# Hawkeye-FineGrained/Hawkeye

Hardware: AMD Instinct MI355X
Metric: images/sec (train fwd+bwd) BCNN VGG-16 448^2 bs64 (higher is better)
Workload: dtype f32; 1 GPU; BCNN_S2: VGG-16 448x448, per-GPU batch 64, 200 classes, SGD momentum 0.9, CE label_smoothing 0.1, full train step; global_batch=64, parallelism=dp1, memory_format=channels_last

## Files before the change

hawkeye_amd/_lib.py:

```python
import ctypes
import os

import torch

_HERE = os.path.dirname(os.path.abspath(__file__))
LIB_PATH = os.path.join(_HERE, 'csrc', 'libhawkeye_hip.so')

c_f = ctypes.c_void_p
c_i = ctypes.c_int
c_sz = ctypes.c_size_t
c_ll = ctypes.c_longlong
c_fl = ctypes.c_float

SIGNATURES = {
    'hk_version': (ctypes.c_char_p, []),
    'hk_tuning_set': (c_i, [ctypes.c_char_p, c_i]),
    'hk_tuning_get': (c_i, [ctypes.c_char_p, ctypes.POINTER(ctypes.c_int)]),
    'hk_bcnn_pool_ws_bytes': (c_sz, [c_i, c_i, c_i]),
    'hk_bcnn_pool_fwd': (c_i, [c_f, c_f, c_f, c_f, c_i, c_i, c_i, c_f, c_sz, c_f]),
    'hk_bcnn_pool_bwd': (c_i, [c_f, c_f, c_f, c_f, c_f, c_f, c_i, c_i, c_i, c_f, c_sz, c_f]),
    'hk_bcnn_pool_bwd_tdot': (c_i, [c_f, c_f, c_f, c_f, c_f, c_f, c_f, c_f, c_i, c_f, c_i, c_i, c_i, c_f, c_sz, c_f]),
    'hk_bcnn_ssqrt_ws_bytes': (c_sz, [c_i, c_i, c_i]),
    'hk_bcnn_ssqrt_pool_fwd': (c_i, [c_f, c_f, c_f, c_i, c_i, c_i, c_f, c_sz, c_f]),
    'hk_bcnn_ssqrt_pool_bwd': (c_i, [c_f, c_f, c_f, c_f, c_f, c_i, c_i, c_i, c_f, c_sz, c_f]),
    'hk_bcnn_ssqrt_pool_fwd_parts': (c_i, [c_f, c_f, c_f, ctypes.c_void_p, c_i, c_i, c_i, c_f]),
    'hk_linear_fwd_ssq': (c_i, [c_f, c_f, c_f, c_f, c_i, c_f, c_f, c_i, c_i, c_i, c_f, c_sz, c_f]),
    'hk_bcnn_ssqrt_pool_bwd_tdot': (c_i, [c_f, c_f, c_f, c_f, c_f, c_f, c_f, c_i, c_i, c_f, c_i, c_i, c_i, c_f, c_sz, c_f]),
    'hk_bcnn_ssqrt_pool_fwd_unscaled': (c_i, [c_f, c_f, c_f, c_i, c_i, c_i, c_f, c_sz, c_f]),
    'hk_bcnn_ssqrt_pool_bwd_unscaled': (c_i, [c_f, c_f, c_f, c_f, c_f, c_i, c_i, c_i, c_f, c_sz, c_f]),
    'hk_bcnn_colsum_norm': (c_i, [c_f, c_f, c_f, c_i, c_i, c_i, c_f, c_sz, c_f]),
    'hk_bcnn_gram_norm': (c_i, [c_f, c_f, c_f, c_i, c_i, c_i, c_f]),
    'hk_bcnn_bwd_gemm': (c_i, [c_f, c_f, c_f, c_f, c_f, c_f, c_i, c_i, c_i, c_f]),
    'hk_bcnn_bwd_rank1': (c_i, [c_f, c_f, c_f, c_f, c_i, c_i, c_i, c_f]),
    'hk_cov_pool_fwd': (c_i, [c_f, c_f, c_f, c_i, c_i, c_i, c_f]),
    'hk_cov_pool_bwd': (c_i, [c_f, c_f, c_f, c_f, c_i, c_i, c_i, c_f]),
    'hk_ns_sqrtm_ws_bytes': (c_sz, [c_i, c_i, c_i, c_i]),
    'hk_ns_sqrtm_fwd': (c_i, [c_f, c_f, c_f, c_f, c_f, c_i, c_i, c_i, c_f, c_sz, c_f]),
    'hk_ns_sqrtm_fwd_sym': (c_i, [c_f, c_f, c_f, c_f, c_f, c_i, c_i, c_i, c_f, c_sz, c_f]),
    'hk_ns_sqrtm_triu_fwd': (c_i, [c_f, c_f, c_f, c_f, c_f, c_f, c_i, c_i, c_i, c_i, c_f, c_sz, c_f]),
    'hk_ns_sqrtm_bwd': (c_i, [c_f, c_f, c_f, c_f, c_f, c_f, c_f, c_i, c_i, c_i, c_f, c_sz, c_f]),
    'hk_ns_sqrtm_bwd_general': (c_i, [c_f, c_f, c_f, c_f, c_f, c_f, c_f, c_i, c_i, c_i, c_f, c_sz, c_f]),
    'hk_triu_vec_fwd': (c_i, [c_f, c_f, c_i, c_i, c_f]),
    'hk_triu_vec_bwd': (c_i, [c_f, c_f, c_i, c_i, c_f]),
    'hk_cbp_plan_bytes': (c_sz, [c_i, c_i]),
    'hk_cbp_plan_build': (c_i, [c_f, c_f, c_f, c_f, c_i, c_i, c_f, c_f]),
    'hk_cbp_plan_destroy': (c_i, [c_f]),
    'hk_cbp_ws_bytes': (c_sz, [c_i, c_i, c_i, c_i]),
    'hk_cbp_fwd': (c_i, [c_f, c_f, c_f, c_f, c_f, c_i, c_i, c_i, c_i, c_f, c_sz, c_f]),
    'hk_cbp_bwd': (c_i, [c_f, c_f, c_f, c_f, c_f, c_f, c_f, c_i, c_i, c_i, c_i, c_f, c_sz, c_f]),
    'hk_trunk_ws_bytes': (c_sz, [c_i]),
    'hk_bias_relu_fwd': (c_i, [c_f, c_f, c_f, c_ll, c_i, c_f]),
    'hk_bias_relu_bwd': (c_i, [c_f, c_f, c_f, c_f, c_f, c_ll, c_i, c_f, c_sz, c_f]),
    'hk_bias_relu_pool_fwd': (c_i, [c_f, c_f, c_f, c_f, c_i, c_i, c_i, c_i, c_f]),
    'hk_bias_relu_pool_bwd': (c_i, [c_f, c_f, c_f, c_f, c_f, c_i, c_i, c_i, c_i, c_f, c_sz, c_f]),
    'hk_conv1_ws_bytes': (c_sz, [c_i]),
    'hk_conv1_bias_relu_fwd': (c_i, [c_f, c_f, c_f, c_f, c_f, c_i, c_i, c_i, c_i, c_i, c_f]),
    'hk_conv1_bias_relu_bwd': (c_i, [c_f, c_f, c_f, c_f, c_f, c_i, c_i, c_i, c_i, c_i, c_f, c_sz, c_f]),
    'hk_conv3x3_wrw_ws_bytes': (c_sz, [c_i, c_i]),
    'hk_conv3x3_wrw': (c_i, [c_f, c_f, c_f, c_i, c_i, c_i, c_i, c_i, c_f, c_sz, c_f]),
    'hk_add_relu_fwd': (c_i, [c_f, c_f, c_ll, c_f]),
    'hk_relu_mask_bwd': (c_i, [c_f, c_f, c_f, c_ll, c_f]),
    'hk_cbp_rect_plan_bytes': (c_sz, [c_i, c_i, c_i]),
    'hk_cbp_rect_plan_build': (c_i, [c_f, c_f, c_i, c_f, c_f, c_i, c_i, c_f, c_f]),
    'hk_cbp_rect_bin_matrix': (c_i, [c_f, c_f, c_f, c_i, c_i, c_i, c_i, c_f]),
    'hk_cbp_rect_unbin_matrix': (c_i, [c_f, c_f, c_f, c_i, c_i, c_i, c_i, c_f]),
    'hk_cbp_rect_loc_fwd': (c_i, [c_f, c_f, c_f, c_f, c_i, c_i, c_i, c_i, c_i, c_f]),
    'hk_cbp_rect_loc_bwd': (c_i, [c_f, c_f, c_f, c_f, c_f, c_f, c_i, c_i, c_i, c_i, c_i, c_f]),
    'hk_att_pool_fwd': (c_i, [c_f, c_f, c_f, c_f, c_i, c_i, c_i, c_f]),
    'hk_att_pool_bwd': (c_i, [c_f, c_f, c_f, c_f, c_f, c_f, c_i, c_i, c_i, c_f]),
    'hk_att_pool3_fwd': (c_i, [c_f] * 8 + [c_i] * 5 + [c_f]),
    'hk_att_pool3_bwd': (c_i, [c_f] * 14 + [c_i] * 5 + [c_f]),
    'hk_att_roi_select3': (c_i, [c_f, c_f, c_f, c_i, c_f, c_f, c_f, c_f, c_i, c_i, c_f, c_fl, c_f, c_f]),
    'hk_att_roi_select': (c_i, [c_f, c_f, c_f, c_i, c_i, c_i, c_i, c_fl, c_i, c_i, c_i, c_i, c_i, c_i, c_fl, c_i, c_f]),
    'hk_roi_crop_resize_fwd': (c_i, [c_f, c_f, c_f, c_f, c_i, c_i, c_i, c_i, c_i, c_f]),
    'hk_roi_crop_resize_bwd': (c_i, [c_f, c_f, c_f, c_f, c_i, c_i, c_i, c_i, c_i, c_f]),
    'hk_roi_boxes': (c_i, [c_f, c_f, c_i, c_f, c_f, c_i, c_f, c_f, c_i, c_f, c_fl, c_f, c_f, c_i, c_f]),
    'hk_osme_gap': (c_i, [c_f, c_f, c_i, c_i, c_i, c_f]),
    'hk_osme_scale_fwd': (c_i, [c_f, c_f, c_f, c_i, c_i, c_i, c_i, c_f]),
    'hk_osme_scale_bwd': (c_i, [c_f, c_f, c_f, c_f, c_f, c_f, c_i, c_i, c_i, c_i, c_f]),
    'hk_linear_ws_bytes': (c_sz, [c_i, c_i, c_i]),
    'hk_linear_fwd': (c_i, [c_f, c_f, c_f, c_f, c_i, c_i, c_i, c_f, c_sz, c_f]),
    'hk_linear_bwd': (c_i, [c_f, c_f, c_f, c_f, c_f, c_f, c_i, c_i, c_i, c_f]),
    'hk_linear_fwd_scaled': (c_i, [c_f, c_f, c_f, c_f, c_f, c_i, c_i, c_i, c_f, c_sz, c_f]),
    'hk_linear_bwd_scaled': (c_i, [c_f, c_f, c_f, c_f, c_f, c_f, c_f, c_i, c_i, c_i, c_f]),
    'hk_npairs_ws_bytes': (c_sz, [c_i, c_i]),
    'hk_npairs_loss': (c_i, [c_f, c_f, c_f, c_f, c_i, c_i, c_i, c_f, c_sz, c_f]),
    'hk_peer_loss_ws_bytes': (c_sz, [c_i, c_i]),
    'hk_peer_loss': (c_i, [c_f, c_f, c_f, ctypes.c_double, c_f, c_f, c_f, c_f, c_i, c_i, c_f, c_sz, c_f]),
    'hk_api_pairs': (c_i, [c_f, c_f, c_f, c_i, c_i, c_f]),
    'hk_api_gather_fwd': (c_i, [c_f, c_f, c_f, c_i, c_i, c_f]),
    'hk_api_gather_bwd': (c_i, [c_f, c_f, c_f, c_i, c_i, c_f]),
    'hk_api_interact_fwd': (c_i, [c_f, c_f, c_f, c_f, c_fl, c_f, c_i, c_i, c_f]),
    'hk_api_interact_bwd': (c_i, [c_f, c_f, c_f, c_f, c_fl, c_f, c_f, c_f, c_i, c_i, c_f]),
    'hk_apinet_loss_ws_bytes': (c_sz, [c_i, c_i]),
    'hk_apinet_loss': (c_i, [c_f, c_f, c_f, c_fl, c_fl, c_f, c_f, c_f, c_i, c_i, c_f, c_sz, c_f]),
    'hk_nts_nms': (c_i, [c_f, c_f, c_f, c_f, c_i, c_i, c_i, ctypes.c_double, c_f]),
    'hk_nts_crop_resize': (c_i, [c_f, c_f, c_f] + [c_i] * 8 + [c_f]),
    'hk_nts_loss_ws_bytes': (c_sz, [c_i, c_i, c_i]),
    'hk_nts_loss': (c_i, [c_f] * 5 + [c_fl] + [c_f] * 5 + [c_i, c_i, c_i, c_f, c_sz, c_f]),
    'hk_crossx_me_fwd': (c_i, [c_f] * 7 + [c_i] * 5 + [c_f]),
    'hk_crossx_me_bwd': (c_i, [c_f] * 12 + [c_i] * 5 + [c_f]),
    'hk_crossx_up_add_fwd': (c_i, [c_f] * 3 + [c_i] * 6 + [c_f]),
    'hk_crossx_up_add_bwd': (c_i, [c_f] * 2 + [c_i] * 6 + [c_f]),
    'hk_crossx_loss_ws_bytes': (c_sz, [c_i] * 6),
    'hk_crossx_loss': (c_i, [c_f] * 7 + [c_fl] * 4 + [c_f] * 7 + [c_i] * 6 + [c_f, c_sz, c_f]),
    'hk_cin_sci_fwd': (c_i, [c_f, c_f, c_f, c_i, c_i, c_i, c_f]),
    'hk_cin_sci_bwd': (c_i, [c_f, c_f, c_f, c_f, c_i, c_f, c_i, c_i, c_i, c_f]),
    'hk_cin_cci_fwd': (c_i, [c_f, c_f, c_f, c_f, c_i, c_i, c_i, c_f]),
    'hk_cin_cci_ws_bytes': (c_sz, [c_i, c_i]),
    'hk_cin_cci_bwd': (c_i, [c_f, c_f, c_f, c_f, c_f, c_f, c_f, c_i, c_i, c_i, c_f, c_sz, c_f]),
    'hk_image_finalize': (c_i, [c_f, c_f, c_f, c_f, c_f, c_i, c_i, c_i, c_i, c_f]),
    'hk_bgemm_f32': (c_i, [c_f, c_i, c_ll, c_i, c_f, c_i, c_ll, c_i, c_f, c_i, c_ll, c_i, c_i, c_i, c_i,
                           c_fl, c_fl, c_fl, c_f]),
    'hk_dcl_head_fwd_ws_bytes': (c_sz, [c_i] * 4),
    'hk_dcl_head_fwd': (c_i, [c_f] * 5 + [c_i] * 4 + [c_f, c_sz, c_f]),
    'hk_dcl_head_bwd_ws_bytes': (c_sz, [c_i] * 4),
    'hk_dcl_head_bwd': (c_i, [c_f] * 8 + [c_i] * 4 + [c_f, c_sz, c_f]),
    'hk_dcl_loss': (c_i, [c_f] * 6 + [c_fl] * 5 + [c_f] * 4 + [c_i] * 4 + [c_f]),
    'hk_dcl_swap_law': (c_i, [c_f] * 6 + [c_i] * 5 + [c_f]),
}

TRUNK_SIGNATURES = {
    'hk_conv3x3_ws_bytes': (c_sz, [c_i, c_i]),
    'hk_conv3x3_fwd': (c_i, [c_f, c_f, c_f, c_i, c_i, c_i, c_i, c_i, c_f, c_sz, c_f]),
    'hk_conv3x3_bwd_data': (c_i, [c_f, c_f, c_f, c_i, c_i, c_i, c_i, c_i, c_f, c_sz, c_f]),
}

TRUNK_EPI_SIGNATURES = {
    'hk_conv3x3_bias_relu_fwd': (c_i, [c_f, c_f, c_f, c_f, c_f, c_i, c_i, c_i, c_i, c_i, c_f, c_sz, c_f]),
    'hk_conv3x3_bias_relu_pool_fwd': (c_i, [c_f, c_f, c_f, c_f, c_f, c_i, c_i, c_i, c_i, c_i, c_f, c_sz, c_f]),
    'hk_conv3x3_masked_ws_bytes': (c_sz, [c_i, c_i, c_i, c_i, c_i]),
    'hk_conv3x3_masked_bwd_data': (c_i, [c_f, c_f, c_f, c_f, c_f, c_i, c_i, c_i, c_i, c_i, c_f, c_sz, c_f]),
}

TRUNK_TILE_SIGNATURES = {
    'hk_conv3x3_tile_plan': (c_i, [c_i, c_i, c_i, c_i, c_f]),
}

TRUNK_POOL_SIGNATURES = {
    'hk_conv3x3_wrw_pooled': (c_i, [c_f, c_f, c_f, c_f, c_f, c_i, c_i, c_i, c_i, c_i, c_f, c_sz, c_f]),
    'hk_conv3x3_wrw_pooled_served': (c_i, [c_i] * 5),
    'hk_conv3x3_wrw_pooled_plan': (c_i, [c_i] * 5 + [c_f]),
}

INTERP_SIGNATURES = {
    'hk_ip_group_fwd_ws_bytes': (c_sz, [c_i] * 5),
    'hk_ip_group_fwd': (c_i, [c_f] * 7 + [c_i] * 5 + [c_f, c_sz, c_f]),
    'hk_ip_group_bwd_ws_bytes': (c_sz, [c_i] * 5),
    'hk_ip_group_bwd': (c_i, [c_f] * 11 + [c_i] * 5 + [c_f, c_sz, c_f]),
    'hk_ip_loss_ws_bytes': (c_sz, [c_i, c_i]),
    'hk_ip_loss': (c_i, [c_f] * 5 + [c_fl] + [c_f] * 3 + [c_i] * 6 + [c_f, c_sz, c_f]),
}

MGE_SIGNATURES = {
    'hk_mge_partpool_fwd_ws_bytes': (c_sz, [c_i] * 5),
    'hk_mge_partpool_fwd': (c_i, [c_f] * 5 + [c_i] * 5 + [c_f, c_sz, c_f]),
    'hk_mge_partpool_bwd': (c_i, [c_f] * 6 + [c_i] * 5 + [c_f]),
    'hk_mge_cam_bbox': (c_i, [c_f] * 4 + [c_i] * 5 + [c_fl, c_i, c_f]),
    'hk_mge_loss_ws_bytes': (c_sz, [c_i, c_i]),
    'hk_mge_loss': (c_i, [c_f, c_f, c_fl, c_f, c_f, c_i, c_i, c_i, c_f, c_sz, c_f]),
}


def attach(lib):
    for name, (res, args) in list(SIGNATURES.items()) + list(TRUNK_SIGNATURES.items()) + list(TRUNK_EPI_SIGNATURES.items()) + \
            list(TRUNK_TILE_SIGNATURES.items()) + list(TRUNK_POOL_SIGNATURES.items()) + list(INTERP_SIGNATURES.items()) + list(MGE_SIGNATURES.items()):
        fn = getattr(lib, name)
        fn.restype = res
        fn.argtypes = args
    return lib


_lib = None


HK_OK, HK_ERR_BAD_ARG, HK_ERR_WORKSPACE, HK_ERR_UNSUPPORTED = 0, -1, -2, -3


class HawkeyeHipError(RuntimeError):
    pass


def load():
    global _lib
    if _lib is not None:
        return _lib
    if not os.path.exists(LIB_PATH):
        raise HawkeyeHipError(
            f'{LIB_PATH} not found: build it with `python -c "import __graft_entry__ as g; g.build()"` '
            f'or `make -C hawkeye_amd/csrc` (there is no CPU fallback for the HIP ops)')
    _lib = attach(ctypes.CDLL(LIB_PATH, mode=ctypes.RTLD_GLOBAL))
    return _lib


def check(rc, what):
    if rc != 0:
        raise HawkeyeHipError(f'{what} failed with code {rc} '
                              f'({"HK_ERR" if rc < 0 else "hipError_t"})')


def ptr(t):
    if t is None:
        return None
    if not t.is_cuda:
        raise HawkeyeHipError('hawkeye_amd ops run on MI355X only: got a CPU tensor (no CPU fallback; '
                              'the CPU reference lives in oracle/ and is test infrastructure)')
    if not (t.is_contiguous() or (t.dim() == 4 and t.is_contiguous(memory_format=torch.channels_last))):
        raise HawkeyeHipError('internal error: non-contiguous tensor handed to the C ABI')
    if t.device.index != torch.cuda.current_device():
        raise HawkeyeHipError(f'tensor lives on {t.device} but the current HIP device is cuda:{torch.cuda.current_device()}: '
                              f'call torch.cuda.set_device({t.device.index}) (one process per GPU) or wrap the call in '
                              f'`with torch.cuda.device(...)`')
    return ctypes.c_void_p(t.data_ptr())


class tuning:

    def __init__(self, **knobs):
        self.knobs = knobs
        self.saved = {}

    def __enter__(self):
        lib = load()
        for name, value in self.knobs.items():
            old = ctypes.c_int(0)
            check(lib.hk_tuning_get(name.encode(), ctypes.byref(old)), f'hk_tuning_get({name})')
            self.saved[name] = old.value
            check(lib.hk_tuning_set(name.encode(), int(value)), f'hk_tuning_set({name})')
        return self

    def __exit__(self, *exc):
        lib = load()
        for name, value in self.saved.items():
            lib.hk_tuning_set(name.encode(), value)
        return False


def stream():
    return ctypes.c_void_p(torch.cuda.current_stream().cuda_stream)
```

hawkeye_amd/csrc/api.hip:

```cpp
#include <cstdlib>
#include <cstring>

#include "hk_bgemm.h"
#include "../../include/hawkeye_hip.h"

namespace hk {

namespace {
struct Knob {
    const char* name;
    const char* env;
    int Tuning::*field;
};
const Knob kKnobs[] = {
    {"bcnn_generic", "HK_BCNN_GENERIC", &Tuning::bcnn_generic}, {"cbp_bin", "HK_CBP_BIN", &Tuning::cbp_bin},
    {"roi_bwd", "HK_ROI_BWD", &Tuning::roi_bwd},                {"linear_slabs", "HK_LINEAR_SLABS", &Tuning::linear_slabs},
    {"ns_tn", "HK_NS_TN", &Tuning::ns_tn},                      {"bwd_v", "HK_BWD_V", &Tuning::bwd_v},
    {"ns_streams", "HK_NS_STREAMS", &Tuning::ns_streams},        {"sched_b", "HK_SCHED_B", &Tuning::sched_b},
    {"ns_sym", "HK_NS_SYM", &Tuning::ns_sym},
    {"lin_walk", "HK_LIN_WALK", &Tuning::lin_walk},           {"bwd_fold", "HK_BWD_FOLD", &Tuning::bwd_fold},
    {"fwd_fold", "HK_FWD_FOLD", &Tuning::fwd_fold},             {"conv_wrw", "HK_CONV_WRW", &Tuning::conv_wrw},
    {"wrw_wgs", "HK_WRW_WGS", &Tuning::wrw_wgs},                {"peer_form", "HK_PEER_FORM", &Tuning::peer_form},
    {"wrw_split", "HK_WRW_SPLIT", &Tuning::wrw_split},          {"wrw_wide", "HK_WRW_WIDE", &Tuning::wrw_wide},
    {"conv_fwd", "HK_CONV_FWD", &Tuning::conv_fwd},             {"conv_bwd_data", "HK_CONV_BWD_DATA", &Tuning::conv_bwd_data},
    {"conv_epi", "HK_CONV_EPI", &Tuning::conv_epi},             {"conv_mfma", "HK_CONV_MFMA", &Tuning::conv_mfma},
    {"wrw_mfma", "HK_WRW_MFMA", &Tuning::wrw_mfma},             {"conv_tile", "HK_CONV_TILE", &Tuning::conv_tile},
    {"wrw_pool", "HK_WRW_POOL", &Tuning::wrw_pool},
};
Tuning from_env() {
    Tuning t;
    for (const Knob& k : kKnobs)
        if (const char* e = getenv(k.env)) t.*(k.field) = atoi(e);
    return t;
}
}

Tuning& tuning() {
    static Tuning t = from_env();
    return t;
}

}

using namespace hk;

extern "C" int hk_tuning_set(const char* name, int value) {
    if (!name) return HK_ERR_BAD_ARG;
    for (const Knob& k : kKnobs)
        if (!strcmp(name, k.name)) {
            tuning().*(k.field) = value;
            return HK_OK;
        }
    return HK_ERR_BAD_ARG;
}

extern "C" int hk_tuning_get(const char* name, int* value) {
    if (!name || !value) return HK_ERR_BAD_ARG;
    for (const Knob& k : kKnobs)
        if (!strcmp(name, k.name)) {
            *value = tuning().*(k.field);
            return HK_OK;
        }
    return HK_ERR_BAD_ARG;
}

extern "C" const char* hk_version(void) { return "hawkeye_hip 0.1 gfx950"; }

extern "C" int hk_bgemm_f32(const float* a, int lda, long long stride_a, int trans_a, const float* b, int ldb,
                            long long stride_b, int trans_b, float* c, int ldc, long long stride_c, int M, int N,
                            int K, int batch, float alpha, float beta, float diag, hk_stream_t stream) {
    if (!a || !b || !c) return HK_ERR_BAD_ARG;
    hipStream_t st = (hipStream_t)stream;
    const LdPlain la = trans_a ? make_plain(a, stride_a, lda, K, M) : make_plain(a, stride_a, lda, M, K);
    const LdPlain lb = trans_b ? make_plain(b, stride_b, ldb, N, K) : make_plain(b, stride_b, ldb, K, N);
    const EpAffine ep = make_affine(c, stride_c, ldc, alpha, nullptr, beta, diag);
    if (!trans_a && !trans_b) return bgemm_launch<true, false>(la, lb, ep, M, N, K, batch, st);
    if (!trans_a && trans_b) return bgemm_launch<true, true>(la, lb, ep, M, N, K, batch, st);
    if (trans_a && !trans_b) return bgemm_launch<false, false>(la, lb, ep, M, N, K, batch, st);
    return bgemm_launch<false, true>(la, lb, ep, M, N, K, batch, st);
}
```

hawkeye_amd/csrc/conv_fwd.hip:

```cpp
#include "hk_common.h"
#include "hk_split_bf16.h"
#include <hk_mfma_bf16.h>
#include "../../include/hawkeye_hip.h"

namespace hk {

constexpr int CF_CO = 64;
constexpr int CF_R = 4;
constexpr int CF_SW = 32;
constexpr int CF_CK = 32;
constexpr int CF_PIX = 80;
constexpr int CF_HW = CF_SW + 2;
constexpr int CF_HPIX = (CF_R + 2) * CF_HW;
constexpr int CF_XPLANE = CF_HPIX * CF_PIX;
constexpr int CF_WPLANE = CF_CO * CF_PIX;
constexpr int CF_WTAP = 3 * CF_WPLANE;
constexpr int CF_LDS = 3 * CF_XPLANE + 2 * CF_WTAP;
constexpr int CF_XF4 = CF_HPIX * (CF_CK / 4);
constexpr int CF_XU = (CF_XF4 + 255) / 256;
constexpr int CF_FLUSH = 3;

constexpr int CF_MF_32 = 0, CF_MF_16 = 1;
constexpr int CF16_PIX = 64;
constexpr int CF16_XPLANE = CF_HPIX * CF16_PIX;
constexpr int CF16_WPLANE = CF_CO * CF16_PIX;
constexpr int CF16_WTAP = 3 * CF16_WPLANE;
constexpr int CF16_LDS = 3 * CF16_XPLANE + 2 * CF16_WTAP;

constexpr int CF_G_4x32 = 0, CF_G_8x16 = 1, CF_G_16x8 = 2;
template <int G>
struct CfGeo {
    static constexpr int TH = G == CF_G_4x32 ? 4 : (G == CF_G_8x16 ? 8 : 16), TW = 128 / TH;
    static constexpr int HR = TH + 2, HC = TW + 2;
    static constexpr int HP = G == CF_G_16x8 ? 16 : HC;
    static constexpr int LPIX = HR * HP;
    static constexpr int XF4 = HR * HC * (CF_CK / 4);
    static constexpr int XU = (XF4 + 255) / 256;
    static constexpr int PBD = G == CF_G_4x32 ? 16 : (G == CF_G_8x16 ? HP : 2 * HP);
    __host__ __device__ static constexpr int trow(bool m32, int wave, int pb, int l) {
        return G == CF_G_4x32 ? wave : (G == CF_G_8x16 ? 2 * wave + (m32 ? l >> 4 : pb) : 4 * wave + 2 * pb + (l >> 3));
    }
    __host__ __device__ static constexpr int tcol(bool m32, int pb, int l) {
        return G == CF_G_4x32 ? (m32 ? l : 16 * pb + l) : (G == CF_G_8x16 ? (m32 ? (l < 16 ? l : (l - 2) & 15) : l) : l & 7);
    }
};
static_assert(CfGeo<CF_G_4x32>::LPIX == CF_HPIX && CfGeo<CF_G_4x32>::XU == CF_XU && CfGeo<CF_G_4x32>::HP == CF_HW, "4 x 32 is the tile above");
constexpr int CF_PLAN_4x32 = 0, CF_PLAN_8x16 = 1, CF_PLAN_MIXED = 2;
template <int MF, int G>
constexpr int cf_xplane() { return CfGeo<G>::LPIX * (MF == CF_MF_32 ? CF_PIX : CF16_PIX); }
template <int MF, int PLAN>
constexpr int cf_lds() {
    return 3 * cf_xplane<MF, PLAN == CF_PLAN_MIXED ? CF_G_16x8 : PLAN>() + 2 * (MF == CF_MF_32 ? CF_WTAP : CF16_WTAP);
}
static_assert(cf_lds<CF_MF_32, CF_PLAN_4x32>() == CF_LDS && cf_lds<CF_MF_16, CF_PLAN_4x32>() == CF16_LDS, "4 x 32 keeps its LDS");
static_assert(cf_lds<CF_MF_32, CF_PLAN_8x16>() <= CF_LDS && cf_lds<CF_MF_16, CF_PLAN_MIXED>() == 79872 && 2 * 79872 <= 160 * 1024,
              "two workgroups per CU with every plan");
#define CF_TAP_BARRIER(n)                                                                                      \
    do {                                                                                                       \
        asm volatile("" ::: "memory");                                         \
        __builtin_amdgcn_s_waitcnt(HK_VMCNT_IMM(n) & ~(15 << 8));                                              \
        __builtin_amdgcn_s_barrier();                                                                          \
        asm volatile("" ::: "memory");                                                                         \
    } while (0)
__host__ __device__ constexpr int cf16_off(int row, int kg) { return row * CF16_PIX + ((kg ^ ((row >> 1) & 2)) << 4); }
constexpr int CF_B128_GROUPS[4][16] = {{0, 1, 2, 3, 12, 13, 14, 15, 20, 21, 22, 23, 24, 25, 26, 27},
                                       {4, 5, 6, 7, 8, 9, 10, 11, 16, 17, 18, 19, 28, 29, 30, 31},
                                       {32, 33, 34, 35, 44, 45, 46, 47, 52, 53, 54, 55, 56, 57, 58, 59},
                                       {36, 37, 38, 39, 40, 41, 42, 43, 48, 49, 50, 51, 60, 61, 62, 63}};
template <int G>
constexpr bool cf16_group_conflict_free(int g) {
    constexpr int LAST = CfGeo<G>::trow(false, 0, 0, 15) * CfGeo<G>::HP + CfGeo<G>::tcol(false, 0, 15);
    for (int base = 0; base + LAST < CfGeo<G>::LPIX; ++base) {
        unsigned seen = 0;
        for (int i = 0; i < 16; ++i) {
            const int lane = CF_B128_GROUPS[g][i], l = lane & 15;
            const int pix = base + CfGeo<G>::trow(false, 0, 0, l) * CfGeo<G>::HP + CfGeo<G>::tcol(false, 0, l);
            const int slot = (cf16_off(pix, lane >> 4) >> 4) & 15;
            if ((seen >> slot) & 1u) return false;
            seen |= 1u << slot;
        }
    }
    return true;
}
template <int G>
constexpr bool cf16_conflict_free() {
    return cf16_group_conflict_free<G>(0) && cf16_group_conflict_free<G>(1) && cf16_group_conflict_free<G>(2) && cf16_group_conflict_free<G>(3);
}
static_assert(cf16_conflict_free<CF_G_4x32>() && cf16_conflict_free<CF_G_8x16>() && cf16_conflict_free<CF_G_16x8>(),
              "every ds_read_b128 lane group of a CF_MF_16 fragment reads 16 different slots, in every geometry at its pitch");
template <int G>
constexpr bool cf32_conflict_free() {
    for (int g = 0; g < 4; ++g)
        for (int base = 0; base + CfGeo<G>::HP + 16 < CfGeo<G>::LPIX; ++base) {
            unsigned seen = 0;
            for (int i = 0; i < 16; ++i) {
                const int lane = CF_B128_GROUPS[g][i], l = lane & 31;
                const int pix = base + CfGeo<G>::trow(true, 0, 0, l) * CfGeo<G>::HP + CfGeo<G>::tcol(true, 0, l);
                const int slot = ((pix * CF_PIX + (lane >> 5) * 16) >> 4) & 15;
                if ((seen >> slot) & 1u) return false;
                seen |= 1u << slot;
            }
        }
    return true;
}
static_assert(cf32_conflict_free<CF_G_4x32>() && cf32_conflict_free<CF_G_8x16>(), "the CF_MF_32 pixel fragment, both geometries");
static_assert(cf16_off(16, 1) == cf16_off(0, 1) + 16 * CF16_PIX && cf16_off(35, 2) == cf16_off(3, 2) + 32 * CF16_PIX,
              "rows 16 and 32 further on are a constant offset away");
static_assert(CF16_WTAP <= CF_WTAP && CF16_WTAP == 3 * 256 * 16, "the workspace holds either image; a weight tile is three loads a thread");

template <int MF>
__global__ __launch_bounds__(256) void conv3x3_wsplit_kernel(const float* __restrict__ w, char* __restrict__ ws, int M, int K,
                                                             int transposed, long long total) {
    const long long i = (long long)blockIdx.x * 256 + threadIdx.x;
    if (i >= total) return;
    const int nchunk = K / CF_CK;
    constexpr int NQ = MF == CF_MF_32 ? 10 : 8;
    const int q = (int)(i % NQ);
    long long r = i / NQ;
    const int co = (int)(r % CF_CO);
    r /= CF_CO;
    const int tap = (int)(r % 9);
    const int chunk = (int)((r / 9) % nchunk), cot = (int)((r / 9) / nchunk);
    const long long m = (long long)cot * CF_CO + co, k0 = (long long)chunk * CF_CK + 4 * q;
    f32x4 v = {0.f, 0.f, 0.f, 0.f};
    if (q < 8) {
        if (!transposed) {
            v = *reinterpret_cast<const f32x4*>(w + (m * 9 + tap) * K + k0);
        } else {
#pragma unroll
            for (int e = 0; e < 4; ++e) v[e] = w[((k0 + e) * 9 + (8 - tap)) * M + m];
        }
    }
    bf16x4 p[3];
    wrs_split(v, p);
    if (MF == CF_MF_32) {
        char* d = ws + (size_t)r * CF_WTAP + co * CF_PIX + q * 8;
#pragma unroll
        for (int s = 0; s < 3; ++s) *reinterpret_cast<bf16x4*>(d + s * CF_WPLANE) = p[s];
    } else {
        char* d = ws + (size_t)r * CF16_WTAP + cf16_off(co, q >> 1) + (q & 1) * 8;
#pragma unroll
        for (int s = 0; s < 3; ++s) *reinterpret_cast<bf16x4*>(d + s * CF16_WPLANE) = p[s];
    }
}

__device__ __forceinline__ bf16x8 cf_frag(const char* p) {
#if defined(__HIP_DEVICE_COMPILE__)
    return *(const __attribute__((address_space(3))) bf16x8*)p;
#else
    bf16x8 f;
    __builtin_memcpy(&f, p, 16);
    return f;
#endif
}

constexpr int CF_EPI_NONE = 0, CF_EPI_RELU = 1, CF_EPI_POOL = 2, CF_EPI_MASK = 3;
constexpr int CF_PARK = CF_CO + 4;
constexpr int CF_DB_RPG = 128;
static_assert(CF_R * CF_SW * CF_PARK * 4 <= CF_LDS, "the parked tile fits the LDS of the main loop");

__device__ __forceinline__ f32x4 cf_relu4(f32x4 v) {
    f32x4 r;
#pragma unroll
    for (int t = 0; t < 4; ++t) r[t] = v[t] < 0.f ? 0.f : v[t];
    return r;
}
__device__ __forceinline__ unsigned cf_sign4(f32x4 r) {
    return (!(r[0] <= 0.f) ? 1u : 0u) | (!(r[1] <= 0.f) ? 2u : 0u) | (!(r[2] <= 0.f) ? 4u : 0u) | (!(r[3] <= 0.f) ? 8u : 0u);
}

template <int EPI, int G>
__device__ __forceinline__ void cf16_epilogue(const f32x4 (&acc4)[4][2], const f32x4 (&sum4)[4][2], float* ldsf, float* __restrict__ y, int H,
                                              int W, int Cout, long long n, int r0, int c0, int cot, int tile, int wave, int tid, int l15,
                                              int kg, const float* __restrict__ bias, uint8_t* __restrict__ mk,
                                              double* __restrict__ part) {
    typedef CfGeo<G> GE;
    const int c4 = Cout / 4;
    bool live[2];
    long long pix[2];
    f32x4 v[4][2];
#pragma unroll
    for (int pb = 0; pb < 2; ++pb) {
        const int row = r0 + GE::trow(false, wave, pb, l15), col = c0 + GE::tcol(false, pb, l15);
        live[pb] = row < H && col < W;
        pix[pb] = (n * H + row) * W + col;
#pragma unroll
        for (int cb = 0; cb < 4; ++cb) v[cb][pb] = sum4[cb][pb] + acc4[cb][pb];
    }
    if (EPI == CF_EPI_RELU || EPI == CF_EPI_POOL) {
        const f32x4* b4 = reinterpret_cast<const f32x4*>(bias + cot * CF_CO + 4 * kg);
#pragma unroll
        for (int cb = 0; cb < 4; ++cb) {
            const f32x4 b = b4[4 * cb];
#pragma unroll
            for (int pb = 0; pb < 2; ++pb) v[cb][pb] = cf_relu4(v[cb][pb] + b);
        }
    }
    if (EPI == CF_EPI_MASK) {
        typedef unsigned u32x4 __attribute__((ext_vector_type(4)));
#pragma unroll
        for (int pb = 0; pb < 2; ++pb) {
            u32x4 mb = {0u, 0u, 0u, 0u};
            if (live[pb]) mb = *reinterpret_cast<const u32x4*>(mk + pix[pb] * c4 + cot * (CF_CO / 4));
#pragma unroll
            for (int cb = 0; cb < 4; ++cb) {
                const unsigned bits = mb[cb] >> (8 * kg);
#pragma unroll
                for (int e = 0; e < 4; ++e) v[cb][pb][e] = ((bits >> e) & 1u) != 0u ? v[cb][pb][e] : 0.f;
            }
        }
    }
    if (EPI != CF_EPI_POOL) {
#pragma unroll
        for (int pb = 0; pb < 2; ++pb)
            if (live[pb]) {
                float* yp = y + pix[pb] * Cout + cot * CF_CO + 4 * kg;
#pragma unroll
                for (int cb = 0; cb < 4; ++cb) *reinterpret_cast<f32x4*>(yp + 16 * cb) = v[cb][pb];
            }
    }
    if (EPI == CF_EPI_RELU) {
        if (mk) {
#pragma unroll
            for (int pb = 0; pb < 2; ++pb) {
                unsigned own = 0;
#pragma unroll
                for (int cb = 0; cb < 4; ++cb) own |= cf_sign4(v[cb][pb]) << (8 * cb);
                unsigned m4 = 0;
#pragma unroll
                for (int j = 0; j < 4; ++j) m4 |= ((__shfl(own, l15 + 16 * j) >> (8 * kg)) & 0xffu) << (8 * j);
                if (live[pb]) *reinterpret_cast<unsigned*>(mk + pix[pb] * c4 + cot * (CF_CO / 4) + 4 * kg) = m4;
            }
        }
    }
    if (EPI == CF_EPI_POOL) {
        float* park = ldsf;
#pragma unroll
        for (int pb = 0; pb < 2; ++pb) {
            float* mine = park + (GE::trow(false, wave, pb, l15) * GE::TW + GE::tcol(false, pb, l15)) * CF_PARK + 4 * kg;
#pragma unroll
            for (int cb = 0; cb < 4; ++cb) *reinterpret_cast<f32x4*>(mine + 16 * cb) = v[cb][pb];
        }
    }
    if (EPI == CF_EPI_MASK) {
        double s[16];
#pragma unroll
        for (int cb = 0; cb < 4; ++cb)
#pragma unroll
            for (int e = 0; e < 4; ++e) s[4 * cb + e] = (double)v[cb][0][e] + (double)v[cb][1][e];
#pragma unroll
        for (int d = 8; d >= 1; d >>= 1) {
            const bool up = (l15 & d) != 0;
#pragma unroll
            for (int i = 0; i < d; ++i) {
                const double send = up ? s[i] : s[i + d], keep = up ? s[i + d] : s[i];
                s[i] = keep + __shfl_xor(send, d);
            }
        }
        double* red = reinterpret_cast<double*>(ldsf);
        red[wave * CF_CO + 16 * (l15 >> 2) + 4 * kg + (l15 & 3)] = s[0];
        __syncthreads();
        if (tid < CF_CO)
            part[(long long)tile * Cout + cot * CF_CO + tid] = ((red[tid] + red[CF_CO + tid]) + red[2 * CF_CO + tid]) + red[3 * CF_CO + tid];
    }
}

template <int EPI, int MF, int G>
__device__ __forceinline__ void conv3x3_split_tile(float* ldsf, const float* __restrict__ x, const char* __restrict__ ws, float* __restrict__ y,
                                                   int H, int W, int Cin, int Cout, long long n, int r0, int c0, int tile, int cot,
                                                   const float* __restrict__ bias, uint8_t* __restrict__ mk, double* __restrict__ part) {
    typedef CfGeo<G> GE;
    constexpr bool M32 = MF == CF_MF_32;
    static_assert(!(M32 && G == CF_G_16x8), "16 x 8 is a geometry of CF_MF_16 only");
    constexpr int XPLANE = cf_xplane<MF, G>(), WTAP = M32 ? CF_WTAP : CF16_WTAP;
    constexpr int XU = GE::XU, XF4 = GE::XF4, HC = GE::HC, HP = GE::HP;
    char* xs = reinterpret_cast<char*>(ldsf);
    char* wb = xs + 3 * XPLANE;
    const int tid = threadIdx.x, lane = tid & 63, l31 = lane & 31, hf = lane >> 5;
    const int l15 = lane & 15, kg = lane >> 4;
    const int wave = __builtin_amdgcn_readfirstlane(tid >> 6);
    const int nchunk = Cin / CF_CK, total = nchunk * 9;
    const float* xi = x + n * H * W * Cin;
    const char* wt = ws + (size_t)cot * total * WTAP + tid * 16;

    long long xoff[XU];
    unsigned xok = 0;
#pragma unroll
    for (int u = 0; u < XU; ++u) {
        const int idx = tid + 256 * u;
        const bool in = idx < XF4;
        const int p = in ? idx >> 3 : 0, hr = p / HC, hc = p - hr * HC;
        const int row = r0 - 1 + hr, col = c0 - 1 + hc;
        if (in && row >= 0 && row < H && col >= 0 && col < W) xok |= 1u << u;
        const int rc = row < 0 ? 0 : (row < H ? row : H - 1), cc = col < 0 ? 0 : (col < W ? col : W - 1);
        xoff[u] = ((long long)rc * W + cc) * Cin + 4 * (idx & 7);
    }
    const int xdst = M32 ? (tid >> 3) * CF_PIX + (tid & 7) * 8 : cf16_off(tid >> 3, (tid & 7) >> 1) + (tid & 1) * 8;
    auto xdst_of = [&](int u) {
        if constexpr (HP == HC) {
            return xdst + u * 32 * (M32 ? CF_PIX : CF16_PIX);
        } else {
            const int p = (tid >> 3) + 32 * u, hr = p / HC;
            return cf16_off(hr * HP + (p - hr * HC), (tid & 7) >> 1) + (tid & 1) * 8;
        }
    };

    f32x4 vx[XU];
    auto load_x = [&](int chunk) {
        const float* b = xi + chunk * CF_CK;
#pragma unroll
        for (int u = 0; u < XU; ++u) HK_LOAD16_ASYNC(vx[u], b + xoff[u]);
    };
    auto load_w = [&](int it, int buf) {
        const char* b = wt + (size_t)it * WTAP;
        char* d = wb + buf * WTAP + wave * 1024;
#pragma unroll
        for (int u = 0; u < 3; ++u) glds16(reinterpret_cast<const float*>(b + 4096 * u), reinterpret_cast<float*>(d + 4096 * u));
        if constexpr (M32) {
            if (wave < 3) glds16(reinterpret_cast<const float*>(b + 3 * 4096), reinterpret_cast<float*>(d + 3 * 4096));
        }
    };
    auto store_x = [&]() {
        const f32x4 zero = {0.f, 0.f, 0.f, 0.f};
#pragma unroll
        for (int u = 0; u < XU; ++u) {
            if (tid + 256 * u < XF4) {
                bf16x4 p[3];
                wrs_split(((xok >> u) & 1) ? vx[u] : zero, p);
                const int d = xdst_of(u);
#pragma unroll
                for (int s = 0; s < 3; ++s) *reinterpret_cast<bf16x4*>(xs + s * XPLANE + d) = p[s];
            }
        }
    };

    f32x16 acc[2], sum[2];
    f32x4 acc4[4][2], sum4[4][2];
    if constexpr (M32) {
#pragma unroll
        for (int cb = 0; cb < 2; ++cb)
#pragma unroll
            for (int i = 0; i < 16; ++i) acc[cb][i] = sum[cb][i] = 0.f;
    } else {
#pragma unroll
        for (int cb = 0; cb < 4; ++cb)
#pragma unroll
            for (int pb = 0; pb < 2; ++pb)
#pragma unroll
                for (int e = 0; e < 4; ++e) acc4[cb][pb][e] = sum4[cb][pb][e] = 0.f;
    }

    load_w(0, 0);
    load_x(0);
    __builtin_amdgcn_s_waitcnt(HK_VMCNT_IMM(0));
#pragma unroll
    for (int u = 0; u < XU; ++u) HK_PIN_LOADED(vx[u]);
    store_x();
    HK_LDS_BARRIER();

    const int aoff = l31 * CF_PIX + hf * 16;
    const int boff = (GE::trow(true, wave, 0, l31) * HP + GE::tcol(true, 0, l31)) * CF_PIX + hf * 16;
    const int bpix = GE::trow(false, wave, 0, l15) * HP + GE::tcol(false, 0, l15);
    int since = 0;
    for (int chunk = 0; chunk < nchunk; ++chunk) {
        const bool more = chunk + 1 < nchunk;
#pragma unroll
        for (int tap = 0; tap < 9; ++tap) {
            const int it = chunk * 9 + tap;
            load_w(it + 1 < total ? it + 1 : it, (it + 1) & 1);
            if (tap == 5) load_x(more ? chunk + 1 : chunk);
            if constexpr (M32) {
            const char* A = wb + (it & 1) * CF_WTAP + aoff;
            const char* B = xs + boff + ((tap / 3) * HP + tap % 3) * CF_PIX;
            bf16x8 a[2][2][3], b[2][3];
#pragma unroll
            for (int ks = 0; ks < 2; ++ks)
#pragma unroll
                for (int s = 0; s < 3; ++s) {
                    b[ks][s] = cf_frag(B + s * XPLANE + ks * 32);
                    a[ks][0][s] = cf_frag(A + s * CF_WPLANE + ks * 32);
                    a[ks][1][s] = cf_frag(A + s * CF_WPLANE + 32 * CF_PIX + ks * 32);
                }
            __builtin_amdgcn_sched_barrier(0);
#pragma unroll
            for (int ks = 0; ks < 2; ++ks)
#pragma unroll
                for (int cb = 0; cb < 2; ++cb) {
                    acc[cb] = __builtin_amdgcn_mfma_f32_32x32x16_bf16(a[ks][cb][1], b[ks][1], acc[cb], 0, 0, 0);
                    acc[cb] = __builtin_amdgcn_mfma_f32_32x32x16_bf16(a[ks][cb][0], b[ks][2], acc[cb], 0, 0, 0);
                    acc[cb] = __builtin_amdgcn_mfma_f32_32x32x16_bf16(a[ks][cb][2], b[ks][0], acc[cb], 0, 0, 0);
                    acc[cb] = __builtin_amdgcn_mfma_f32_32x32x16_bf16(a[ks][cb][0], b[ks][1], acc[cb], 0, 0, 0);
                    acc[cb] = __builtin_amdgcn_mfma_f32_32x32x16_bf16(a[ks][cb][1], b[ks][0], acc[cb], 0, 0, 0);
                    acc[cb] = __builtin_amdgcn_mfma_f32_32x32x16_bf16(a[ks][cb][0], b[ks][0], acc[cb], 0, 0, 0);
                }
            } else {
                const char* A = wb + (it & 1) * CF16_WTAP + cf16_off(l15, kg);
                const int bp = bpix + (tap / 3) * HP + tap % 3;
                const char* Bp[2];
                Bp[0] = xs + cf16_off(bp, kg);
                Bp[1] = GE::PBD % 16 == 0 ? Bp[0] + GE::PBD * CF16_PIX : xs + cf16_off(bp + GE::PBD, kg);
                bf16x8 a[4][3], b[2][3];
#pragma unroll
                for (int s = 0; s < 3; ++s) {
#pragma unroll
                    for (int pb = 0; pb < 2; ++pb) b[pb][s] = cf_frag(Bp[pb] + s * XPLANE);
#pragma unroll
                    for (int cb = 0; cb < 4; ++cb) a[cb][s] = cf_frag(A + s * CF16_WPLANE + cb * 16 * CF16_PIX);
                }
                __builtin_amdgcn_sched_barrier(0);
                constexpr int PA[6] = {1, 0, 2, 0, 1, 0}, PB[6] = {1, 2, 0, 1, 0, 0};
#pragma unroll
                for (int pr = 0; pr < 6; ++pr)
#pragma unroll
                    for (int cb = 0; cb < 4; ++cb)
#pragma unroll
                        for (int pb = 0; pb < 2; ++pb) acc4[cb][pb] = mfma_f32_16x16x32_bf16(a[cb][PA[pr]], b[pb][PB[pr]], acc4[cb][pb]);
            }
            if (tap == 5) CF_TAP_BARRIER(XU);
            else CF_TAP_BARRIER(0);
            if (tap == 6) {
#pragma unroll
                for (int u = 0; u < XU; ++u) HK_PIN_LOADED(vx[u]);
            }
            if (tap == 8 && more) {
                store_x();
                HK_LDS_BARRIER();
            }
        }
        if (++since == CF_FLUSH) {
            if constexpr (M32) {
#pragma unroll
                for (int cb = 0; cb < 2; ++cb) {
                    sum[cb] += acc[cb];
#pragma unroll
                    for (int i = 0; i < 16; ++i) acc[cb][i] = 0.f;
                }
            } else {
#pragma unroll
                for (int cb = 0; cb < 4; ++cb)
#pragma unroll
                    for (int pb = 0; pb < 2; ++pb) {
                        sum4[cb][pb] += acc4[cb][pb];
#pragma unroll
                        for (int e = 0; e < 4; ++e) acc4[cb][pb][e] = 0.f;
                    }
            }
            since = 0;
        }
    }
    if constexpr (!M32) {
        cf16_epilogue<EPI, G>(acc4, sum4, ldsf, y, H, W, Cout, n, r0, c0, cot, tile, wave, tid, l15, kg, bias, mk, part);
        if (EPI != CF_EPI_POOL) return;
    }
    const int trow = GE::trow(true, wave, 0, l31), tcol = GE::tcol(true, 0, l31);
    const int row = r0 + trow, col = c0 + tcol;
    if (EPI == CF_EPI_NONE) {
        if (row < H && col < W) {
            float* yp = y + ((n * H + row) * W + col) * Cout + cot * CF_CO + 4 * hf;
#pragma unroll
            for (int cb = 0; cb < 2; ++cb)
#pragma unroll
                for (int j = 0; j < 4; ++j) {
                    f32x4 v;
#pragma unroll
                    for (int e = 0; e < 4; ++e) v[e] = sum[cb][4 * j + e] + acc[cb][4 * j + e];
                    *reinterpret_cast<f32x4*>(yp + cb * 32 + 8 * j) = v;
                }
        }
        return;
    }
    const bool live = row < H && col < W;
    const long long pix = (n * H + row) * W + col;
    const int c4 = Cout / 4;
    f32x4 v[2][4];
    if constexpr (M32) {
#pragma unroll
    for (int cb = 0; cb < 2; ++cb)
#pragma unroll
        for (int j = 0; j < 4; ++j)
#pragma unroll
            for (int e = 0; e < 4; ++e) v[cb][j][e] = sum[cb][4 * j + e] + acc[cb][4 * j + e];
    }
    if (M32 && (EPI == CF_EPI_RELU || EPI == CF_EPI_POOL)) {
        const f32x4* b4 = reinterpret_cast<const f32x4*>(bias + cot * CF_CO + 4 * hf);
#pragma unroll
        for (int cb = 0; cb < 2; ++cb)
#pragma unroll
            for (int j = 0; j < 4; ++j) v[cb][j] = cf_relu4(v[cb][j] + b4[8 * cb + 2 * j]);
    }
    if (EPI == CF_EPI_RELU) {
        if (live) {
            float* yp = y + pix * Cout + cot * CF_CO + 4 * hf;
#pragma unroll
            for (int cb = 0; cb < 2; ++cb)
#pragma unroll
                for (int j = 0; j < 4; ++j) *reinterpret_cast<f32x4*>(yp + cb * 32 + 8 * j) = v[cb][j];
        }
        if (mk) {
            unsigned own[2];
#pragma unroll
            for (int cb = 0; cb < 2; ++cb) {
                own[cb] = 0;
#pragma unroll
                for (int j = 0; j < 4; ++j) own[cb] |= cf_sign4(v[cb][j]) << (8 * j);
            }
            const unsigned theirs0 = __shfl_xor(own[0], 32), theirs1 = __shfl_xor(own[1], 32);
            const unsigned ev = hf ? theirs1 : own[0], od = hf ? own[1] : theirs0;
            unsigned long long m8 = 0;
#pragma unroll
            for (int k = 0; k < 4; ++k)
                m8 |= ((unsigned long long)((ev >> (8 * k)) & 0xffu) << (16 * k)) | ((unsigned long long)((od >> (8 * k)) & 0xffu) << (16 * k + 8));
            if (live) *reinterpret_cast<unsigned long long*>(mk + pix * c4 + cot * (CF_CO / 4) + 8 * hf) = m8;
        }
    }
    if (EPI == CF_EPI_POOL) {
        float* park = ldsf;
        if constexpr (M32) {
        float* mine = park + (trow * GE::TW + tcol) * CF_PARK + 4 * hf;
#pragma unroll
        for (int cb = 0; cb < 2; ++cb)
#pragma unroll
            for (int j = 0; j < 4; ++j) *reinterpret_cast<f32x4*>(mine + cb * 32 + 8 * j) = v[cb][j];
        }
        __syncthreads();
        constexpr int TW = GE::TW, PW = TW / 2;
        const int q = tid & 15;
        const int Ho = H / 2, Wo = W / 2;
#pragma unroll
        for (int u = 0; u < 2; ++u) {
            const int pp = (tid >> 4) + 16 * u, pr = pp / PW, pc = pp % PW;
            const float* src = park + (2 * pr * TW + 2 * pc) * CF_PARK + 4 * q;
            f32x4 m = *reinterpret_cast<const f32x4*>(src);
            unsigned code = 0;
#pragma unroll
            for (int k = 1; k < 4; ++k) {
                const f32x4 a = *reinterpret_cast<const f32x4*>(src + ((k >> 1) * TW + (k & 1)) * CF_PARK);
#pragma unroll
                for (int t = 0; t < 4; ++t) {
                    const bool take = (a[t] > m[t]) || (a[t] != a[t]);
                    m[t] = take ? a[t] : m[t];
                    code = take ? ((code & ~(3u << (2 * t))) | ((unsigned)k << (2 * t))) : code;
                }
            }
            unsigned t1 = __shfl_xor(code, 1);
            unsigned c2 = (q & 1) ? (t1 | (code << 8)) : (code | (t1 << 8));
            unsigned t2 = __shfl_xor(c2, 2);
            unsigned c4b = (q & 2) ? (t2 | (c2 << 16)) : (c2 | (t2 << 16));
            unsigned t4 = __shfl_xor(c4b, 4);
            const unsigned long long lo = (q & 4) ? t4 : c4b, hi = (q & 4) ? c4b : t4;
            const int ho = r0 / 2 + pr, wo = c0 / 2 + pc;
            if (ho < Ho && wo < Wo) {
                const long long opix = (n * Ho + ho) * Wo + wo;
                *reinterpret_cast<f32x4*>(y + opix * Cout + cot * CF_CO + 4 * q) = m;
                if ((q & 7) == 0) *reinterpret_cast<unsigned long long*>(mk + opix * c4 + cot * (CF_CO / 4) + q) = lo | (hi << 32);
            }
        }
    }
    if (EPI == CF_EPI_MASK) {
        typedef unsigned u32x4 __attribute__((ext_vector_type(4)));
        u32x4 mb = {0u, 0u, 0u, 0u};
        if (live) mb = *reinterpret_cast<const u32x4*>(mk + pix * c4 + cot * (CF_CO / 4));
        double s[32];
#pragma unroll
        for (int cb = 0; cb < 2; ++cb)
#pragma unroll
            for (int j = 0; j < 4; ++j) {
                const unsigned bits = mb[2 * cb + (j >> 1)] >> (8 * (2 * (j & 1) + hf));
#pragma unroll
                for (int e = 0; e < 4; ++e) {
                    v[cb][j][e] = ((bits >> e) & 1u) != 0u ? v[cb][j][e] : 0.f;
                    s[16 * cb + 4 * j + e] = v[cb][j][e];
                }
            }
        if (live) {
            float* yp = y + pix * Cout + cot * CF_CO + 4 * hf;
#pragma unroll
            for (int cb = 0; cb < 2; ++cb)
#pragma unroll
                for (int j = 0; j < 4; ++j) *reinterpret_cast<f32x4*>(yp + cb * 32 + 8 * j) = v[cb][j];
        }
#pragma unroll
        for (int d = 16; d >= 1; d >>= 1) {
            const bool up = (l31 & d) != 0;
#pragma unroll
            for (int i = 0; i < d; ++i) {
                const double send = up ? s[i] : s[i + d], keep = up ? s[i + d] : s[i];
                s[i] = keep + __shfl_xor(send, d);
            }
        }
        double* red = reinterpret_cast<double*>(ldsf);
        red[wave * CF_CO + 32 * (l31 >> 4) + 8 * ((l31 >> 2) & 3) + 4 * hf + (l31 & 3)] = s[0];
        __syncthreads();
        if (tid < CF_CO)
            part[(long long)tile * Cout + cot * CF_CO + tid] = ((red[tid] + red[CF_CO + tid]) + red[2 * CF_CO + tid]) + red[3 * CF_CO + tid];
    }
}

template <int EPI, int MF, int PLAN>
__global__ __launch_bounds__(256, 2) void conv3x3_split_kernel(const float* __restrict__ x, const char* __restrict__ ws,
                                                               float* __restrict__ y, int H, int W, int Cin, int Cout, int nstrips,
                                                               int nrb, int ntiles, const float* __restrict__ bias,
                                                               uint8_t* __restrict__ mk, double* __restrict__ part, int nstripsB, int tpi) {
    HK_DYN_LDS16(ldsf);
    int tile, cot;
    if (!xcd_map(blockIdx.x, ntiles, Cout / CF_CO, tile, cot)) return;
    if constexpr (PLAN != CF_PLAN_MIXED) {
        typedef CfGeo<PLAN> GE;
        const int strip = tile % nstrips, tr = tile / nstrips;
        const int rb = tr % nrb;
        const long long n = tr / nrb;
        conv3x3_split_tile<EPI, MF, PLAN>(ldsf, x, ws, y, H, W, Cin, Cout, n, rb * GE::TH, strip * GE::TW, tile, cot, bias, mk, part);
    } else {
        const long long n = tile / tpi;
        const int t = tile % tpi, nA = nrb * nstrips;
        if (t < nA) {
            conv3x3_split_tile<EPI, MF, CF_G_8x16>(ldsf, x, ws, y, H, W, Cin, Cout, n, (t / nstrips) * 8, (t % nstrips) * 16, tile, cot, bias, mk,
                                                   part);
        } else {
            const int tb = t - nA;
            conv3x3_split_tile<EPI, MF, CF_G_16x8>(ldsf, x, ws, y, H, W, Cin, Cout, n, (tb / nstripsB) * 16, nstrips * 16 + (tb % nstripsB) * 8,
                                                   tile, cot, bias, mk, part);
        }
    }
}

template <int Q, typename OUT>
__global__ __launch_bounds__(64 * Q) void conv3x3_colsum_kernel(const double* __restrict__ part, int nrows, int nel, int rpg,
                                                                OUT* __restrict__ out) {
    __shared__ double red[Q][64];
    const int l = threadIdx.x & 63, q = threadIdx.x >> 6;
    const int e = blockIdx.x * 64 + l;
    const int beg = blockIdx.y * rpg, end = beg + rpg < nrows ? beg + rpg : nrows;
    double s = 0.0;
    if (e < nel) {
        int k = beg + q;
        for (; k + 7 * Q < end; k += 8 * Q) {
            double t[8];
#pragma unroll
            for (int u = 0; u < 8; ++u) t[u] = part[(long long)(k + Q * u) * nel + e];
#pragma unroll
            for (int u = 0; u < 8; ++u) s += t[u];
        }
        for (; k < end; k += Q) s += part[(long long)k * nel + e];
    }
    red[q][l] = s;
    __syncthreads();
    if (q == 0 && e < nel) {
        double t = red[0][l];
        for (int k = 1; k < Q; ++k) t += red[k][l];
        out[(long long)blockIdx.y * nel + e] = (OUT)t;
    }
}

struct CfPlan {
    int plan;
    long long tpi;
    int nrb, nstrips;
    int nrbB, nstripsB;
};
static CfPlan conv3x3_plan(int H, int W, int mf, int knob) {
    auto cdiv = [](long long a, long long b) { return (int)((a + b - 1) / b); };
    CfPlan c[3];
    c[0] = {CF_PLAN_4x32, 0, cdiv(H, 4), cdiv(W, 32), 0, 0};
    c[1] = {CF_PLAN_8x16, 0, cdiv(H, 8), cdiv(W, 16), 0, 0};
    c[2] = {CF_PLAN_MIXED, 0, cdiv(H, 8), W / 16, cdiv(H, 16), cdiv(W % 16, 8)};
    for (CfPlan& p : c) p.tpi = (long long)p.nrb * p.nstrips + (long long)p.nrbB * p.nstripsB;
    const int ncand = mf == CF_MF_16 ? 3 : 2;
    if (knob == 0) return c[0];
    int best = 0;
    for (int i = 1; i < ncand; ++i)
        if (c[i].tpi < c[best].tpi) best = i;
    return c[best];
}

template <int EPI, int MF, int PLAN>
static int conv3x3_run_on(const float* x, const float* w, float* y, int N, int H, int W, int K, int M, bool transposed, void* ws,
                          hipStream_t stream, const float* bias, uint8_t* mk, double* part, const CfPlan& pl) {
    constexpr int LDS = cf_lds<MF, PLAN>();
    const long long ntiles = N * pl.tpi;
    const int ncot = M / CF_CO;
    if ((ntiles + NXCD) * ncot > 0x7fffffffll) return HK_ERR_UNSUPPORTED;
    const long long total = (long long)ncot * (K / CF_CK) * 9 * CF_CO * (MF == CF_MF_32 ? 10 : 8);
    hipLaunchKernelGGL(conv3x3_wsplit_kernel<MF>, dim3((unsigned)((total + 255) / 256)), dim3(256), 0, stream, w, (char*)ws, M, K,
                       transposed ? 1 : 0, total);
    HK_LAUNCH_CHECK();
    HK_ALLOW_BIG_LDS((conv3x3_split_kernel<EPI, MF, PLAN>), LDS);
    hipLaunchKernelGGL((conv3x3_split_kernel<EPI, MF, PLAN>), dim3((unsigned)xcd_grid((int)ntiles, ncot)), dim3(256), LDS, stream, x,
                       (const char*)ws, y, H, W, K, M, pl.nstrips, pl.nrb, (int)ntiles, bias, mk, part, pl.nstripsB, (int)pl.tpi);
    HK_LAUNCH_CHECK();
    return HK_OK;
}
static bool conv3x3_mfma16_wins(int N, int H, int W, int K, int M) {
    (void)N, (void)H, (void)W, (void)K, (void)M;
    return true;
}
static int conv3x3_mf(int N, int H, int W, int K, int M) {
    const int knob = tuning().conv_mfma;
    return knob == 1 || (knob < 0 && conv3x3_mfma16_wins(N, H, W, K, M)) ? CF_MF_16 : CF_MF_32;
}
template <int EPI>
static int conv3x3_run(const float* x, const float* w, float* y, int N, int H, int W, int K, int M, bool transposed, void* ws,
                       hipStream_t stream, const float* bias = nullptr, uint8_t* mk = nullptr, double* part = nullptr) {
    const int mf = conv3x3_mf(N, H, W, K, M);
    const CfPlan pl = conv3x3_plan(H, W, mf, tuning().conv_tile);
    if (pl.tpi > 0x7fffffffll) return HK_ERR_UNSUPPORTED;
    if (mf == CF_MF_16) {
        if (pl.plan == CF_PLAN_MIXED) return conv3x3_run_on<EPI, CF_MF_16, CF_PLAN_MIXED>(x, w, y, N, H, W, K, M, transposed, ws, stream, bias, mk, part, pl);
        if (pl.plan == CF_PLAN_8x16) return conv3x3_run_on<EPI, CF_MF_16, CF_PLAN_8x16>(x, w, y, N, H, W, K, M, transposed, ws, stream, bias, mk, part, pl);
        return conv3x3_run_on<EPI, CF_MF_16, CF_PLAN_4x32>(x, w, y, N, H, W, K, M, transposed, ws, stream, bias, mk, part, pl);
    }
    if (pl.plan == CF_PLAN_8x16) return conv3x3_run_on<EPI, CF_MF_32, CF_PLAN_8x16>(x, w, y, N, H, W, K, M, transposed, ws, stream, bias, mk, part, pl);
    return conv3x3_run_on<EPI, CF_MF_32, CF_PLAN_4x32>(x, w, y, N, H, W, K, M, transposed, ws, stream, bias, mk, part, pl);
}

static int conv3x3_check(const float* x, const float* w, float* y, int N, int H, int W, int Cin, int Cout, void* ws, size_t ws_bytes,
                         int knob) {
    if (!x || !w || !y || N <= 0 || H <= 0 || W <= 0 || Cin <= 0 || Cout <= 0) return HK_ERR_BAD_ARG;
    if (!ws || ws_bytes < hk_conv3x3_ws_bytes(Cin, Cout)) return HK_ERR_WORKSPACE;
    if (Cin % 64 != 0 || Cout % 64 != 0 || (long long)Cout * 9 * Cin > 0x7fffffffll || !aligned16(x) || !aligned16(w) || !aligned16(y) ||
        !aligned16(ws) || knob == 0)
        return HK_ERR_UNSUPPORTED;
    return HK_OK;
}

static long long conv3x3_tiles(int N, int H, int W) {
    return (long long)N * (((long long)H + CF_R - 1) / CF_R) * (((long long)W + CF_SW - 1) / CF_SW);
}
static long long conv3x3_groups(long long ntiles) { return ntiles > CF_DB_RPG ? (ntiles + CF_DB_RPG - 1) / CF_DB_RPG : 0; }

}

using namespace hk;

extern "C" size_t hk_conv3x3_ws_bytes(int Cin, int Cout) {
    if (Cin <= 0 || Cout <= 0) return 0;
    const size_t a = ((size_t)Cout + 63) / 64 * (((size_t)Cin + 31) / 32), b = ((size_t)Cin + 63) / 64 * (((size_t)Cout + 31) / 32);
    return (a > b ? a : b) * 9 * CF_WTAP;
}

extern "C" int hk_conv3x3_fwd(const float* x, const float* w, float* y, int N, int H, int W, int Cin, int Cout, void* ws, size_t ws_bytes,
                              hk_stream_t stream) {
    const int rc = conv3x3_check(x, w, y, N, H, W, Cin, Cout, ws, ws_bytes, tuning().conv_fwd);
    return rc != HK_OK ? rc : conv3x3_run<CF_EPI_NONE>(x, w, y, N, H, W, Cin, Cout, false, ws, (hipStream_t)stream);
}

extern "C" int hk_conv3x3_bwd_data(const float* dy, const float* w, float* dx, int N, int H, int W, int Cin, int Cout, void* ws,
                                   size_t ws_bytes, hk_stream_t stream) {
    const int rc = conv3x3_check(dy, w, dx, N, H, W, Cin, Cout, ws, ws_bytes, tuning().conv_bwd_data);
    return rc != HK_OK ? rc : conv3x3_run<CF_EPI_NONE>(dy, w, dx, N, H, W, Cout, Cin, true, ws, (hipStream_t)stream);
}

extern "C" int hk_conv3x3_bias_relu_fwd(const float* x, const float* w, const float* bias, float* y, uint8_t* mask, int N, int H, int W,
                                        int Cin, int Cout, void* ws, size_t ws_bytes, hk_stream_t stream) {
    if (!bias) return HK_ERR_BAD_ARG;
    const int rc = conv3x3_check(x, w, y, N, H, W, Cin, Cout, ws, ws_bytes, tuning().conv_fwd);
    if (rc != HK_OK) return rc;
    if (!aligned16(bias) || (((uintptr_t)mask) & 7) != 0 || tuning().conv_epi < 1) return HK_ERR_UNSUPPORTED;
    return conv3x3_run<CF_EPI_RELU>(x, w, y, N, H, W, Cin, Cout, false, ws, (hipStream_t)stream, bias, mask);
}

extern "C" int hk_conv3x3_bias_relu_pool_fwd(const float* x, const float* w, const float* bias, float* p, uint8_t* argmax, int N, int H,
                                             int W, int Cin, int Cout, void* ws, size_t ws_bytes, hk_stream_t stream) {
    if (!bias || !argmax) return HK_ERR_BAD_ARG;
    const int rc = conv3x3_check(x, w, p, N, H, W, Cin, Cout, ws, ws_bytes, tuning().conv_fwd);
    if (rc != HK_OK) return rc;
    if (H % 2 != 0 || W % 2 != 0 || !aligned16(bias) || (((uintptr_t)argmax) & 7) != 0 || tuning().conv_epi < 1) return HK_ERR_UNSUPPORTED;
    return conv3x3_run<CF_EPI_POOL>(x, w, p, N, H, W, Cin, Cout, false, ws, (hipStream_t)stream, bias, argmax);
}

extern "C" size_t hk_conv3x3_masked_ws_bytes(int N, int H, int W, int Cin, int Cout) {
    if (N <= 0 || H <= 0 || W <= 0 || Cin <= 0 || Cout <= 0) return 0;
    const long long ntiles = conv3x3_tiles(N, H, W);
    return hk_conv3x3_ws_bytes(Cin, Cout) + (size_t)(ntiles + conv3x3_groups(ntiles)) * Cin * sizeof(double);
}

extern "C" int hk_conv3x3_tile_plan(int N, int H, int W, int mf, int* out) {
    if (!out || N <= 0 || H <= 0 || W <= 0 || (mf != CF_MF_32 && mf != CF_MF_16)) return HK_ERR_BAD_ARG;
    const CfPlan pl = conv3x3_plan(H, W, mf, tuning().conv_tile);
    if (pl.tpi > 0x7fffffffll) return HK_ERR_UNSUPPORTED;
    const bool mixed = pl.plan == CF_PLAN_MIXED;
    const int th = pl.plan == CF_PLAN_4x32 ? 4 : 8;
    const bool a = pl.nstrips > 0;
    int r[2][5] = {{th, 128 / th, pl.nrb, pl.nstrips, 0}, {16, 8, pl.nrbB, pl.nstripsB, 16 * pl.nstrips}};
    const int first = mixed && !a ? 1 : 0, nreg = mixed && a && pl.nstripsB > 0 ? 2 : 1;
    out[0] = (int)pl.tpi;
    out[1] = nreg;
    for (int i = 0; i < 2; ++i)
        for (int k = 0; k < 5; ++k) out[2 + 5 * i + k] = i < nreg ? r[first + i][k] : 0;
    return HK_OK;
}

extern "C" int hk_conv3x3_masked_bwd_data(const float* dy, const float* w, const uint8_t* mask, float* dx, float* dbias, int N, int H, int W,
                                          int Cin, int Cout, void* ws, size_t ws_bytes, hk_stream_t stream) {
    if (!mask || !dbias) return HK_ERR_BAD_ARG;
    const int rc = conv3x3_check(dy, w, dx, N, H, W, Cin, Cout, ws, ws_bytes, tuning().conv_bwd_data);
    if (rc != HK_OK) return rc;
    if (ws_bytes < hk_conv3x3_masked_ws_bytes(N, H, W, Cin, Cout)) return HK_ERR_WORKSPACE;
    if (!aligned16(mask) || tuning().conv_epi < 2) return HK_ERR_UNSUPPORTED;
    const long long ntiles = N * conv3x3_plan(H, W, conv3x3_mf(N, H, W, Cout, Cin), tuning().conv_tile).tpi, ngroups = conv3x3_groups(ntiles);
    if (ntiles > conv3x3_tiles(N, H, W) || ntiles > 0x7fffffffll || ngroups > 65535) return HK_ERR_UNSUPPORTED;
    double* part = reinterpret_cast<double*>((char*)ws + hk_conv3x3_ws_bytes(Cin, Cout));
    double* grp = part + ntiles * Cin;
    const int rc2 = conv3x3_run<CF_EPI_MASK>(dy, w, dx, N, H, W, Cout, Cin, true, ws, (hipStream_t)stream, nullptr, const_cast<uint8_t*>(mask), part);
    if (rc2 != HK_OK) return rc2;
    const dim3 cols((unsigned)(Cin / 64));
    if (ngroups > 0) {
        hipLaunchKernelGGL((conv3x3_colsum_kernel<16, double>), dim3(cols.x, (unsigned)ngroups), dim3(1024), 0, (hipStream_t)stream,
                           (const double*)part, (int)ntiles, Cin, CF_DB_RPG, grp);
        HK_LAUNCH_CHECK();
        hipLaunchKernelGGL((conv3x3_colsum_kernel<16, float>), cols, dim3(1024), 0, (hipStream_t)stream, (const double*)grp, (int)ngroups, Cin,
                           (int)ngroups, dbias);
    } else {
        hipLaunchKernelGGL((conv3x3_colsum_kernel<16, float>), cols, dim3(1024), 0, (hipStream_t)stream, (const double*)part, (int)ntiles, Cin,
                           (int)ntiles, dbias);
    }
    HK_LAUNCH_CHECK();
    return HK_OK;
}
```

hawkeye_amd/csrc/hk_common.h:

```cpp
#pragma once
#include <hip/hip_runtime.h>
#include <stdint.h>
#include <stddef.h>
#include <mutex>

typedef float f32x2 __attribute__((ext_vector_type(2)));
typedef float f32x4 __attribute__((ext_vector_type(4)));
typedef float f32x16 __attribute__((ext_vector_type(16)));

#define HK_OK 0
#define HK_ERR_BAD_ARG (-1)
#define HK_ERR_WORKSPACE (-2)
#define HK_ERR_UNSUPPORTED (-3)

#include <hk_isa.h>

#define HK_VMCNT_IMM(n) (((n) & 15) | (((n) >> 4) << 14) | (7 << 4) | (15 << 8))
#define HK_VM_BARRIER(n)                                                                                       \
    do {                                                                                                       \
        asm volatile("" ::: "memory");                                         \
        __builtin_amdgcn_s_waitcnt(HK_VMCNT_IMM(n));                                                           \
        __builtin_amdgcn_s_barrier();                                                                          \
        asm volatile("" ::: "memory");                                                                         \
    } while (0)

#define HK_LAUNCH_CHECK()                                 \
    do {                                                  \
        hipError_t e__ = hipGetLastError();               \
        if (e__ != hipSuccess) return (int)e__;           \
    } while (0)

namespace hk {

struct Tuning {
    int bcnn_generic = 0;
    int cbp_bin = -1;
    int roi_bwd = 0;
    int linear_slabs = 0;
    int ns_tn = 0;
    int bwd_v = 0;
    int ns_streams = 1;
    int ns_sym = 1;
    int lin_walk = -1;
    int fwd_fold = 0;
    int bwd_fold = 0;
    int sched_b = 0;
    int conv_wrw = 1;
    int wrw_wgs = 0;
    int wrw_split = -1;
    int wrw_wide = 1;
    int wrw_mfma = -1;
    int wrw_pool = -1;
    int conv_fwd = -1;
    int conv_bwd_data = -1;
    int conv_epi = 2;
    int conv_mfma = -1;
    int conv_tile = -1;
    int peer_form = 0;
};
Tuning& tuning();

constexpr int HK_MAX_AUX = 3;
struct AuxQueue {
    hipStream_t aux[HK_MAX_AUX] = {nullptr, nullptr, nullptr};
    hipEvent_t fork = nullptr, join[HK_MAX_AUX] = {nullptr, nullptr, nullptr};
    bool ok = false;
    std::mutex busy;
};
inline AuxQueue* aux_queue(hipStream_t st) {
    static AuxQueue tab[16];
    static std::once_flag once[16];
    int dev = 0, sdev = 0;
    if (hipGetDevice(&dev) != hipSuccess || dev < 0 || dev >= 16) return nullptr;
    if (st != nullptr && (hipStreamGetDevice(st, &sdev) != hipSuccess || sdev != dev)) return nullptr;
    AuxQueue& a = tab[dev];
    std::call_once(once[dev], [&a]() {
        bool good = hipEventCreateWithFlags(&a.fork, hipEventDisableTiming) == hipSuccess;
        for (int i = 0; i < HK_MAX_AUX && good; ++i)
            good = hipStreamCreateWithFlags(&a.aux[i], hipStreamNonBlocking) == hipSuccess &&
                   hipEventCreateWithFlags(&a.join[i], hipEventDisableTiming) == hipSuccess;
        if (!good) {
            for (int i = 0; i < HK_MAX_AUX; ++i) {
                if (a.join[i]) (void)hipEventDestroy(a.join[i]);
                if (a.aux[i]) (void)hipStreamDestroy(a.aux[i]);
                a.join[i] = nullptr; a.aux[i] = nullptr;
            }
            if (a.fork) (void)hipEventDestroy(a.fork);
            a.fork = nullptr;
        }
        a.ok = good;
    });
    return a.ok ? &a : nullptr;
}
class AuxScope {
  public:
    AuxScope(hipStream_t st, int n) : st_(st) {
        if (n <= 0) return;
        if (n > HK_MAX_AUX) n = HK_MAX_AUX;
        q_ = aux_queue(st);
        if (!q_) return;
        q_->busy.lock();
        bool good = hipEventRecord(q_->fork, st_) == hipSuccess;
        for (int i = 0; i < n && good; ++i) good = hipStreamWaitEvent(q_->aux[i], q_->fork, 0) == hipSuccess;
        if (good) {
            n_ = n;
        } else {
            q_->busy.unlock();
            q_ = nullptr;
        }
    }
    AuxScope(const AuxScope&) = delete;
    AuxScope& operator=(const AuxScope&) = delete;
    ~AuxScope() { (void)join(); }
    int count() const { return n_; }
    hipStream_t aux(int i) const { return q_->aux[i]; }
    int join() {
        if (!n_) return HK_OK;
        hipError_t e = hipSuccess;
        for (int i = 0; i < n_; ++i) {
            hipError_t r = hipEventRecord(q_->join[i], q_->aux[i]);
            if (r == hipSuccess) r = hipStreamWaitEvent(st_, q_->join[i], 0);
            if (e == hipSuccess) e = r;
        }
        n_ = 0;
        q_->busy.unlock();
        q_ = nullptr;
        return e == hipSuccess ? HK_OK : (int)e;
    }

  private:
    hipStream_t st_;
    int n_ = 0;
    AuxQueue* q_ = nullptr;
};

constexpr int WAVE = 64;
constexpr int NXCD = 8;

template <int AUX = 0>
__device__ __forceinline__ void glds16(const float* g, float* l) {
    __builtin_amdgcn_global_load_lds((const __attribute__((address_space(1))) void*)g,
                                     (__attribute__((address_space(3))) void*)l, 16, 0, AUX);
}

__device__ __forceinline__ void glds4(const float* g, float* l) {
    __builtin_amdgcn_global_load_lds((const __attribute__((address_space(1))) void*)g,
                                     (__attribute__((address_space(3))) void*)l, 4, 0, 0);
}

__device__ __forceinline__ float wave_sum(float v) {
#pragma unroll
    for (int o = 32; o > 0; o >>= 1) v += __shfl_xor(v, o, 64);
    return v;
}

__device__ __forceinline__ float wave_max(float v) {
#pragma unroll
    for (int o = 32; o > 0; o >>= 1) v = fmaxf(v, __shfl_xor(v, o, 64));
    return v;
}

template <int NW>
__device__ __forceinline__ float block_sum(float v, float* red) {
    v = wave_sum(v);
    const int w = threadIdx.x >> 6;
    __syncthreads();
    if ((threadIdx.x & 63) == 0) red[w] = v;
    __syncthreads();
    float s = 0.f;
#pragma unroll
    for (int i = 0; i < NW; ++i) s += red[i];
    return s;
}

__host__ __device__ __forceinline__ int xcd_grid(int nb, int tiles) {
    return (nb >= NXCD) ? NXCD * ((nb + NXCD - 1) / NXCD) * tiles : nb * tiles;
}
__device__ __forceinline__ bool xcd_map(int bid, int nb, int tiles, int& sample, int& tile) {
    if (nb >= NXCD) {
        const int xcd = bid % NXCD, slot = bid / NXCD;
        sample = xcd + NXCD * (slot / tiles);
        tile = slot % tiles;
    } else {
        sample = bid / tiles;
        tile = bid % tiles;
    }
    return sample < nb;
}

__host__ __forceinline__ bool aligned16(const void* p) { return (((uintptr_t)p) & 15) == 0; }

#define HK_ALLOW_BIG_LDS(fn, bytes)                                                                            \
    do {                                                                                                       \
        static size_t have_[32] = {0};                                                                         \
        int dev_ = 0;                                                                                          \
        if (hipGetDevice(&dev_) != hipSuccess || dev_ < 0 || dev_ > 31) dev_ = 0;                             \
        if ((size_t)(bytes) > 64 * 1024 && (size_t)(bytes) > have_[dev_]) {                                    \
            const hipError_t e_ = hipFuncSetAttribute(reinterpret_cast<const void*>(fn),                      \
                                                      hipFuncAttributeMaxDynamicSharedMemorySize, (int)(bytes)); \
            if (e_ != hipSuccess) return (int)e_;                                                              \
            have_[dev_] = (size_t)(bytes);                                                                     \
        }                                                                                                      \
    } while (0)

}
```

hawkeye_amd/csrc/trunk.hip:

```cpp
#include "hk_common.h"
#include "hk_partial_sum.h"
#include "../../include/hawkeye_hip.h"

namespace hk {

constexpr int TRUNK_PART_BLOCKS = 1024;

__device__ __forceinline__ f32x4 relu4(f32x4 v) {
    f32x4 r;
#pragma unroll
    for (int t = 0; t < 4; ++t) r[t] = v[t] < 0.f ? 0.f : v[t];
    return r;
}

template <bool MASK>
__global__ __launch_bounds__(256) void bias_relu_fwd_kernel(float* __restrict__ x, const float* __restrict__ b,
                                                            uint8_t* __restrict__ mask, long long n4, int c4) {
    f32x4* x4 = reinterpret_cast<f32x4*>(x);
    const f32x4* b4 = reinterpret_cast<const f32x4*>(b);
    const long long stride = (long long)gridDim.x * 256;
    for (long long i = (long long)blockIdx.x * 256 + threadIdx.x; i < n4; i += 4 * stride) {
        f32x4 v[4];
#pragma unroll
        for (int u = 0; u < 4; ++u)
            if (i + u * stride < n4) v[u] = x4[i + u * stride];
#pragma unroll
        for (int u = 0; u < 4; ++u) {
            const long long j = i + u * stride;
            if (j < n4) {
                const f32x4 r = relu4(v[u] + b4[(int)(j % c4)]);
                x4[j] = r;
                if (MASK) mask[j] = (uint8_t)((!(r[0] <= 0.f) ? 1 : 0) | (!(r[1] <= 0.f) ? 2 : 0) | (!(r[2] <= 0.f) ? 4 : 0) | (!(r[3] <= 0.f) ? 8 : 0));
            }
        }
    }
}

__device__ __forceinline__ void trunk_db_partial(f32x4 acc, float* __restrict__ part, int c4) {
    __shared__ f32x4 red[256];
    const int tid = threadIdx.x;
    red[tid] = acc;
    __syncthreads();
    if (tid < c4) {
        f32x4 s = red[tid];
        for (int g = 1; g < 256 / c4; ++g) s += red[tid + g * c4];
        reinterpret_cast<f32x4*>(part + (long long)blockIdx.x * 4 * c4)[tid] = s;
    }
}

template <bool MASK>
__global__ __launch_bounds__(256) void bias_relu_bwd_kernel(const float* dy, const float* __restrict__ y,
                                                            const uint8_t* __restrict__ mask, float* dx,
                                                            float* __restrict__ part, long long rows, long long rpb, int c4) {
    const int tid = threadIdx.x, q = tid % c4, r0 = tid / c4, rstep = 256 / c4;
    const long long rbeg = (long long)blockIdx.x * rpb, rend = rbeg + rpb < rows ? rbeg + rpb : rows;
    const f32x4* dy4 = reinterpret_cast<const f32x4*>(dy);
    const f32x4* y4 = reinterpret_cast<const f32x4*>(y);
    f32x4* dx4 = reinterpret_cast<f32x4*>(dx);
    f32x4 acc = (f32x4){0.f, 0.f, 0.f, 0.f};
    for (long long r = rbeg + r0; r < rend; r += 4 * rstep) {
        f32x4 g[4], v[4];
        unsigned mk[4];
#pragma unroll
        for (int u = 0; u < 4; ++u) {
            const long long rr = r + u * rstep;
            if (rr < rend) {
                g[u] = dy4[rr * c4 + q];
                if (MASK) mk[u] = mask[rr * c4 + q];
                else v[u] = y4[rr * c4 + q];
            }
        }
#pragma unroll
        for (int u = 0; u < 4; ++u) {
            const long long rr = r + u * rstep;
            if (rr < rend) {
                f32x4 d;
#pragma unroll
                for (int t = 0; t < 4; ++t)
                    d[t] = (MASK ? ((mk[u] >> t) & 1u) != 0u : !(v[u][t] <= 0.f)) ? g[u][t] : 0.f;
                dx4[rr * c4 + q] = d;
                acc += d;
            }
        }
    }
    trunk_db_partial(acc, part, c4);
}

__global__ __launch_bounds__(256) void trunk_db_final_kernel(const float* __restrict__ part, int nblk, int C, float* __restrict__ db) {
    __shared__ float red[16][17];
    const int cl = threadIdx.x & 15, g = threadIdx.x >> 4;
    const int c = blockIdx.x * 16 + cl;
    float s = 0.f;
    if (c < C) {
        int k = g;
        for (; k + 7 * 16 < nblk; k += 8 * 16) {
            float v[8];
#pragma unroll
            for (int u = 0; u < 8; ++u) v[u] = part[(long long)(k + 16 * u) * C + c];
#pragma unroll
            for (int u = 0; u < 8; ++u) s += v[u];
        }
        for (; k < nblk; k += 16) s += part[(long long)k * C + c];
    }
    red[g][cl] = s;
    __syncthreads();
    if (g == 0 && c < C) {
        float t = red[0][cl];
        for (int k = 1; k < 16; ++k) t += red[k][cl];
        db[c] = t;
    }
}

__global__ __launch_bounds__(256) void bias_relu_pool_fwd_kernel(const float* __restrict__ x, const float* __restrict__ b,
                                                                 float* __restrict__ p, uint8_t* __restrict__ am, long long n4out,
                                                                 int c4, int Wo, int Ho) {
    const long long i = (long long)blockIdx.x * 256 + threadIdx.x;
    if (i >= n4out) return;
    const int q = (int)(i % c4);
    const long long pix = i / c4;
    const int wo = (int)(pix % Wo);
    const long long nh = pix / Wo;
    const int ho = (int)(nh % Ho);
    const long long n = nh / Ho;
    const long long W = 2ll * Wo;
    const f32x4* x4 = reinterpret_cast<const f32x4*>(x);
    const long long base = ((n * 2 * Ho + 2 * ho) * W + 2 * wo) * c4 + q;
    f32x4 v[4];
    v[0] = x4[base];
    v[1] = x4[base + c4];
    v[2] = x4[base + W * c4];
    v[3] = x4[base + W * c4 + c4];
    const f32x4 bb = reinterpret_cast<const f32x4*>(b)[q];
    f32x4 m = relu4(v[0] + bb);
    unsigned code = 0;
#pragma unroll
    for (int k = 1; k < 4; ++k) {
        const f32x4 a = relu4(v[k] + bb);
#pragma unroll
        for (int t = 0; t < 4; ++t) {
            const bool take = (a[t] > m[t]) || (a[t] != a[t]);
            m[t] = take ? a[t] : m[t];
            code = take ? ((code & ~(3u << (2 * t))) | ((unsigned)k << (2 * t))) : code;
        }
    }
    reinterpret_cast<f32x4*>(p)[i] = m;
    am[i] = (uint8_t)code;
}

__global__ __launch_bounds__(256) void bias_relu_pool_bwd_kernel(const float* __restrict__ dp, const float* __restrict__ p,
                                                                 const uint8_t* __restrict__ am, float* __restrict__ dx,
                                                                 float* __restrict__ part, long long npix, long long ppb, int c4,
                                                                 int Wo, int Ho) {
    const int tid = threadIdx.x, q = tid % c4, r0 = tid / c4, rstep = 256 / c4;
    const long long pbeg = (long long)blockIdx.x * ppb, pend = pbeg + ppb < npix ? pbeg + ppb : npix;
    const f32x4* dp4 = reinterpret_cast<const f32x4*>(dp);
    const f32x4* p4 = reinterpret_cast<const f32x4*>(p);
    f32x4* dx4 = reinterpret_cast<f32x4*>(dx);
    const long long W = 2ll * Wo;
    f32x4 acc = (f32x4){0.f, 0.f, 0.f, 0.f};
    for (long long pix = pbeg + r0; pix < pend; pix += 2 * rstep) {
        f32x4 g[2], v[2];
        unsigned code[2];
#pragma unroll
        for (int u = 0; u < 2; ++u) {
            const long long pp = pix + u * rstep;
            if (pp < pend) { g[u] = dp4[pp * c4 + q]; v[u] = p4[pp * c4 + q]; code[u] = am[pp * c4 + q]; }
        }
#pragma unroll
        for (int u = 0; u < 2; ++u) {
            const long long pp = pix + u * rstep;
            if (pp >= pend) continue;
            const int wo = (int)(pp % Wo);
            const long long nh = pp / Wo;
            const int ho = (int)(nh % Ho);
            const long long n = nh / Ho;
            const long long base = ((n * 2 * Ho + 2 * ho) * W + 2 * wo) * c4 + q;
            f32x4 d;
#pragma unroll
            for (int t = 0; t < 4; ++t) d[t] = !(v[u][t] <= 0.f) ? g[u][t] : 0.f;
            acc += d;
            f32x4 o[4];
#pragma unroll
            for (int k = 0; k < 4; ++k)
#pragma unroll
                for (int t = 0; t < 4; ++t) o[k][t] = ((code[u] >> (2 * t)) & 3u) == (unsigned)k ? d[t] : 0.f;
            dx4[base] = o[0];
            dx4[base + c4] = o[1];
            dx4[base + W * c4] = o[2];
            dx4[base + W * c4 + c4] = o[3];
        }
    }
    trunk_db_partial(acc, part, c4);
}

__global__ __launch_bounds__(256) void add_relu_fwd_kernel(float* __restrict__ a, const float* __restrict__ b, long long n4) {
    f32x4* a4 = reinterpret_cast<f32x4*>(a);
    const f32x4* b4 = reinterpret_cast<const f32x4*>(b);
    const long long stride = (long long)gridDim.x * 256;
    for (long long i = (long long)blockIdx.x * 256 + threadIdx.x; i < n4; i += 4 * stride) {
        f32x4 u[4], v[4];
#pragma unroll
        for (int k = 0; k < 4; ++k)
            if (i + k * stride < n4) { u[k] = a4[i + k * stride]; v[k] = b4[i + k * stride]; }
#pragma unroll
        for (int k = 0; k < 4; ++k)
            if (i + k * stride < n4) a4[i + k * stride] = relu4(u[k] + v[k]);
    }
}

__global__ __launch_bounds__(256) void relu_mask_bwd_kernel(const float* __restrict__ dy, const float* __restrict__ y,
                                                            float* __restrict__ g, long long n4) {
    const f32x4* d4 = reinterpret_cast<const f32x4*>(dy);
    const f32x4* y4 = reinterpret_cast<const f32x4*>(y);
    f32x4* g4 = reinterpret_cast<f32x4*>(g);
    const long long stride = (long long)gridDim.x * 256;
    for (long long i = (long long)blockIdx.x * 256 + threadIdx.x; i < n4; i += 4 * stride) {
        f32x4 u[4], v[4];
#pragma unroll
        for (int k = 0; k < 4; ++k)
            if (i + k * stride < n4) { u[k] = d4[i + k * stride]; v[k] = y4[i + k * stride]; }
#pragma unroll
        for (int k = 0; k < 4; ++k)
            if (i + k * stride < n4) {
                f32x4 r;
#pragma unroll
                for (int t = 0; t < 4; ++t) r[t] = !(v[k][t] <= 0.f) ? u[k][t] : 0.f;
                g4[i + k * stride] = r;
            }
    }
}

static inline bool trunk_c_ok(int C) {
    return C >= 4 && C % 4 == 0 && C / 4 <= 256 && 256 % (C / 4) == 0;
}
static inline int trunk_blocks(long long rows) {
    long long b = (rows + 63) / 64;
    return (int)(b < 1 ? 1 : (b > TRUNK_PART_BLOCKS ? TRUNK_PART_BLOCKS : b));
}

}

using namespace hk;

extern "C" size_t hk_trunk_ws_bytes(int C) { return C > 0 ? (size_t)TRUNK_PART_BLOCKS * C * sizeof(float) : 0; }

extern "C" int hk_bias_relu_fwd(float* x, const float* bias, uint8_t* mask, long long rows, int C, hk_stream_t stream) {
    if (!x || !bias || rows <= 0 || C <= 0) return HK_ERR_BAD_ARG;
    if (C % 4 != 0 || !aligned16(x) || !aligned16(bias)) return HK_ERR_UNSUPPORTED;
    const long long n4 = rows * (C / 4);
    long long blocks = (n4 + 1023) / 1024;
    if (blocks > 8192) blocks = 8192;
    if (mask) hipLaunchKernelGGL(bias_relu_fwd_kernel<true>, dim3((unsigned)blocks), dim3(256), 0, (hipStream_t)stream, x, bias, mask, n4, C / 4);
    else hipLaunchKernelGGL(bias_relu_fwd_kernel<false>, dim3((unsigned)blocks), dim3(256), 0, (hipStream_t)stream, x, bias, mask, n4, C / 4);
    HK_LAUNCH_CHECK();
    return HK_OK;
}

extern "C" int hk_bias_relu_bwd(const float* dy, const float* y, const uint8_t* mask, float* dx, float* dbias, long long rows, int C,
                                void* ws, size_t ws_bytes, hk_stream_t stream) {
    if (!dy || (!y && !mask) || !dx || !dbias || rows <= 0 || C <= 0) return HK_ERR_BAD_ARG;
    if (!trunk_c_ok(C) || !aligned16(dy) || (!mask && !aligned16(y)) || !aligned16(dx)) return HK_ERR_UNSUPPORTED;
    if (!ws || ws_bytes < hk_trunk_ws_bytes(C)) return HK_ERR_WORKSPACE;
    const int nblk = trunk_blocks(rows);
    const long long rpb = (rows + nblk - 1) / nblk;
    if (mask) hipLaunchKernelGGL(bias_relu_bwd_kernel<true>, dim3(nblk), dim3(256), 0, (hipStream_t)stream, dy, y, mask, dx, (float*)ws, rows, rpb, C / 4);
    else hipLaunchKernelGGL(bias_relu_bwd_kernel<false>, dim3(nblk), dim3(256), 0, (hipStream_t)stream, dy, y, mask, dx, (float*)ws, rows, rpb, C / 4);
    HK_LAUNCH_CHECK();
    hipLaunchKernelGGL(trunk_db_final_kernel, dim3((C + 15) / 16), dim3(256), 0, (hipStream_t)stream, (const float*)ws, nblk, C, dbias);
    HK_LAUNCH_CHECK();
    return HK_OK;
}

extern "C" int hk_bias_relu_pool_fwd(const float* x, const float* bias, float* p, uint8_t* argmax, int N, int H, int W, int C,
                                     hk_stream_t stream) {
    if (!x || !bias || !p || !argmax || N <= 0 || H <= 0 || W <= 0 || C <= 0) return HK_ERR_BAD_ARG;
    if (C % 4 != 0 || H % 2 != 0 || W % 2 != 0 || !aligned16(x) || !aligned16(bias) || !aligned16(p)) return HK_ERR_UNSUPPORTED;
    const long long n4out = (long long)N * (H / 2) * (W / 2) * (C / 4);
    if ((n4out + 255) / 256 > 0x7fffffffll) return HK_ERR_UNSUPPORTED;
    hipLaunchKernelGGL(bias_relu_pool_fwd_kernel, dim3((unsigned)((n4out + 255) / 256)), dim3(256), 0, (hipStream_t)stream, x, bias, p,
                       argmax, n4out, C / 4, W / 2, H / 2);
    HK_LAUNCH_CHECK();
    return HK_OK;
}

extern "C" int hk_bias_relu_pool_bwd(const float* dp, const float* p, const uint8_t* argmax, float* dx, float* dbias, int N, int H,
                                     int W, int C, void* ws, size_t ws_bytes, hk_stream_t stream) {
    if (!dp || !p || !argmax || !dx || !dbias || N <= 0 || H <= 0 || W <= 0 || C <= 0) return HK_ERR_BAD_ARG;
    if (!trunk_c_ok(C) || H % 2 != 0 || W % 2 != 0 || !aligned16(dp) || !aligned16(p) || !aligned16(dx)) return HK_ERR_UNSUPPORTED;
    if (!ws || ws_bytes < hk_trunk_ws_bytes(C)) return HK_ERR_WORKSPACE;
    const long long npix = (long long)N * (H / 2) * (W / 2);
    const int nblk = trunk_blocks(npix);
    const long long ppb = (npix + nblk - 1) / nblk;
    hipLaunchKernelGGL(bias_relu_pool_bwd_kernel, dim3(nblk), dim3(256), 0, (hipStream_t)stream, dp, p, argmax, dx, (float*)ws, npix,
                       ppb, C / 4, W / 2, H / 2);
    HK_LAUNCH_CHECK();
    hipLaunchKernelGGL(trunk_db_final_kernel, dim3((C + 15) / 16), dim3(256), 0, (hipStream_t)stream, (const float*)ws, nblk, C, dbias);
    HK_LAUNCH_CHECK();
    return HK_OK;
}

extern "C" int hk_add_relu_fwd(float* a, const float* b, long long n, hk_stream_t stream) {
    if (!a || !b || n <= 0) return HK_ERR_BAD_ARG;
    if (n % 4 != 0 || !aligned16(a) || !aligned16(b)) return HK_ERR_UNSUPPORTED;
    long long blocks = (n / 4 + 1023) / 1024;
    if (blocks > 8192) blocks = 8192;
    hipLaunchKernelGGL(add_relu_fwd_kernel, dim3((unsigned)blocks), dim3(256), 0, (hipStream_t)stream, a, b, n / 4);
    HK_LAUNCH_CHECK();
    return HK_OK;
}

extern "C" int hk_relu_mask_bwd(const float* dy, const float* y, float* g, long long n, hk_stream_t stream) {
    if (!dy || !y || !g || n <= 0) return HK_ERR_BAD_ARG;
    if (n % 4 != 0 || !aligned16(dy) || !aligned16(y) || !aligned16(g)) return HK_ERR_UNSUPPORTED;
    long long blocks = (n / 4 + 1023) / 1024;
    if (blocks > 8192) blocks = 8192;
    hipLaunchKernelGGL(relu_mask_bwd_kernel, dim3((unsigned)blocks), dim3(256), 0, (hipStream_t)stream, dy, y, g, n / 4);
    HK_LAUNCH_CHECK();
    return HK_OK;
}

namespace hk {


constexpr int C1_OUT = 64;

template <int CIN>
__global__ __launch_bounds__(256) void conv1_fwd_kernel(const float* __restrict__ x, const float* __restrict__ wt,
                                                        const float* __restrict__ bias, float* __restrict__ y,
                                                        uint8_t* __restrict__ mask, long long npix, int H, int W) {
    constexpr int NT = 9 * CIN;
    __shared__ __attribute__((aligned(16))) float tile[4][64][68];
    const int tid = threadIdx.x, lane = tid & 63, wave = tid >> 6;
    const long long p0 = (long long)blockIdx.x * 256;
    const long long p = p0 + tid;
    const bool live = p < npix;
    const long long pc = live ? p : npix - 1;
    const int w_ = (int)(pc % W);
    const long long nh = pc / W;
    const int h_ = (int)(nh % H);
    float xv[NT];
#pragma unroll
    for (int kh = 0; kh < 3; ++kh) {
        const int hh = h_ + kh - 1;
        const bool rok = hh >= 0 && hh < H;
        const float* row = x + ((nh - h_ + (rok ? hh : h_)) * W) * CIN;
#pragma unroll
        for (int kw = 0; kw < 3; ++kw) {
            const int ww = w_ + kw - 1;
            const bool ok = rok && ww >= 0 && ww < W;
            const float* px = row + (long long)(ok ? ww : w_) * CIN;
#pragma unroll
            for (int c = 0; c < CIN; ++c) {
                const float v = px[c];
                xv[(kh * 3 + kw) * CIN + c] = ok ? v : 0.f;
            }
        }
    }
    float acc[C1_OUT];
#pragma unroll
    for (int o = 0; o < C1_OUT; ++o) acc[o] = 0.f;
#pragma unroll
    for (int t = 0; t < NT; ++t) {
#pragma unroll
        for (int o = 0; o < C1_OUT; ++o) acc[o] = fmaf(xv[t], wt[t * C1_OUT + o], acc[o]);
    }
    float (*T)[68] = tile[wave];
#pragma unroll
    for (int o4 = 0; o4 < C1_OUT / 4; ++o4) {
        f32x4 v;
#pragma unroll
        for (int j = 0; j < 4; ++j) {
            const float s = acc[4 * o4 + j] + bias[4 * o4 + j];
            v[j] = s < 0.f ? 0.f : s;
        }
        *reinterpret_cast<f32x4*>(&T[lane][4 * o4]) = v;
    }
    HK_WAVE_SYNC();
    const long long pw = p0 + 64 * wave;
#pragma unroll
    for (int i = 0; i < 16; ++i) {
        const int pl = 4 * i + (lane >> 4), q = lane & 15;
        const f32x4 v = *reinterpret_cast<const f32x4*>(&T[pl][4 * q]);
        if (pw + pl < npix) {
            reinterpret_cast<f32x4*>(y)[(pw + pl) * 16 + q] = v;
            if (mask) mask[(pw + pl) * 16 + q] = (uint8_t)((!(v[0] <= 0.f) ? 1 : 0) | (!(v[1] <= 0.f) ? 2 : 0) | (!(v[2] <= 0.f) ? 4 : 0) | (!(v[3] <= 0.f) ? 8 : 0));
        }
    }
}

template <int CIN>
__global__ __launch_bounds__(256) void conv1_bwd_kernel(const float* __restrict__ dy, const uint8_t* __restrict__ mask,
                                                        const float* __restrict__ x, float* __restrict__ part, long long nrows,
                                                        int H, int W) {
    constexpr int NT = 9 * CIN;
    static_assert(NT + 1 <= 32, "taps + the ones column fit one 32-wide MFMA tile");
    constexpr int UN = 8;
    __shared__ float red[4][NT + 1][64];
    const int lane = threadIdx.x & 63, l31 = lane & 31, hf = lane >> 5;
    const int wave = __builtin_amdgcn_readfirstlane(threadIdx.x >> 6);
    const bool is_tap = l31 < NT, is_one = l31 == NT;
    const int kh = is_tap ? l31 / (3 * CIN) : 1, kw = is_tap ? (l31 / CIN) % 3 : 1, c = is_tap ? l31 % CIN : 0;
    f32x16 acc0, acc1;
#pragma unroll
    for (int i = 0; i < 16; ++i) { acc0[i] = 0.f; acc1[i] = 0.f; }
    const long long nwaves = (long long)gridDim.x * 4;
    for (long long r = (long long)blockIdx.x * 4 + wave; r < nrows; r += nwaves) {
        const int h_ = (int)(r % H);
        const bool rowok = is_tap && (kh == 0 ? h_ > 0 : (kh == 2 ? h_ + 1 < H : true));
        const float* xb = x + ((r + (rowok ? kh - 1 : 0)) * (long long)W) * CIN + c;
        const float* dyr = dy + r * (long long)W * C1_OUT + l31;
        const uint8_t* mr = mask + r * (long long)W * (C1_OUT / 4) + (l31 >> 2);
        for (int w0 = 0; w0 < W; w0 += 2 * UN) {
            float a0[UN], a1[UN], b[UN];
            unsigned m0[UN], m1[UN];
#pragma unroll
            for (int u = 0; u < UN; ++u) {
                const int w_ = w0 + 2 * u + hf;
                const int wc = w_ < W ? w_ : W - 1;
                a0[u] = dyr[(long long)wc * C1_OUT];
                a1[u] = dyr[(long long)wc * C1_OUT + 32];
                m0[u] = mr[(long long)wc * (C1_OUT / 4)];
                m1[u] = mr[(long long)wc * (C1_OUT / 4) + 8];
                const int ww = w_ + kw - 1;
                const bool okb = rowok && w_ < W && ww >= 0 && ww < W;
                const float v = xb[(long long)(okb ? ww : wc) * CIN];
                b[u] = okb ? v : ((is_one && w_ < W) ? 1.0f : 0.f);
            }
#pragma unroll
            for (int u = 0; u < UN; ++u) {
                const bool in = w0 + 2 * u + hf < W;
                const float g0 = (in && ((m0[u] >> (l31 & 3)) & 1u)) ? a0[u] : 0.f;
                const float g1 = (in && ((m1[u] >> (l31 & 3)) & 1u)) ? a1[u] : 0.f;
                acc0 = __builtin_amdgcn_mfma_f32_32x32x2f32(g0, b[u], acc0, 0, 0, 0);
                acc1 = __builtin_amdgcn_mfma_f32_32x32x2f32(g1, b[u], acc1, 0, 0, 0);
            }
        }
    }
    if (l31 <= NT) {
#pragma unroll
        for (int i = 0; i < 16; ++i) {
            const int o = 8 * (i >> 2) + 4 * hf + (i & 3);
            red[wave][l31][o] = acc0[i];
            red[wave][l31][32 + o] = acc1[i];
        }
    }
    __syncthreads();
    float* pb = part + (long long)blockIdx.x * (NT + 1) * 64;
    for (int e = threadIdx.x; e < (NT + 1) * 64; e += 256) {
        const int t = e >> 6, o = e & 63;
        pb[e] = (red[0][t][o] + red[1][t][o]) + (red[2][t][o] + red[3][t][o]);
    }
}


constexpr int C1_BWD_BLOCKS = 1024;

}

using namespace hk;

extern "C" size_t hk_conv1_ws_bytes(int Cin) {
    return Cin > 0 ? (size_t)C1_BWD_BLOCKS * (9 * (Cin > 3 ? 3 : Cin) + 1) * 64 * sizeof(float) : 0;
}

extern "C" int hk_conv1_bias_relu_fwd(const float* x, const float* wt, const float* bias, float* y, uint8_t* mask, int N, int H, int W,
                                      int Cin, int Cout, hk_stream_t stream) {
    if (!x || !wt || !bias || !y || N <= 0 || H <= 0 || W <= 0 || Cin <= 0 || Cout <= 0) return HK_ERR_BAD_ARG;
    if (Cin > 3 || Cout != C1_OUT || !aligned16(y)) return HK_ERR_UNSUPPORTED;
    const long long npix = (long long)N * H * W;
    const long long blocks = (npix + 255) / 256;
    if (blocks > 0x7fffffffll) return HK_ERR_UNSUPPORTED;
    const dim3 grid((unsigned)blocks);
    switch (Cin) {
        case 1: hipLaunchKernelGGL(conv1_fwd_kernel<1>, grid, dim3(256), 0, (hipStream_t)stream, x, wt, bias, y, mask, npix, H, W); break;
        case 2: hipLaunchKernelGGL(conv1_fwd_kernel<2>, grid, dim3(256), 0, (hipStream_t)stream, x, wt, bias, y, mask, npix, H, W); break;
        default: hipLaunchKernelGGL(conv1_fwd_kernel<3>, grid, dim3(256), 0, (hipStream_t)stream, x, wt, bias, y, mask, npix, H, W); break;
    }
    HK_LAUNCH_CHECK();
    return HK_OK;
}

extern "C" int hk_conv1_bias_relu_bwd(const float* dy, const uint8_t* mask, const float* x, float* dwt, float* dbias, int N, int H, int W,
                                      int Cin, int Cout, void* ws, size_t ws_bytes, hk_stream_t stream) {
    if (!dy || !mask || !x || !dwt || !dbias || N <= 0 || H <= 0 || W <= 0 || Cin <= 0 || Cout <= 0) return HK_ERR_BAD_ARG;
    if (!ws || ws_bytes < hk_conv1_ws_bytes(Cin)) return HK_ERR_WORKSPACE;
    if (Cin > 3 || Cout != C1_OUT) return HK_ERR_UNSUPPORTED;
    const long long nrows = (long long)N * H;
    long long nblk = (nrows + 3) / 4;
    if (nblk > C1_BWD_BLOCKS) nblk = C1_BWD_BLOCKS;
    float* part = (float*)ws;
    switch (Cin) {
        case 1: hipLaunchKernelGGL(conv1_bwd_kernel<1>, dim3((unsigned)nblk), dim3(256), 0, (hipStream_t)stream, dy, mask, x, part, nrows, H, W); break;
        case 2: hipLaunchKernelGGL(conv1_bwd_kernel<2>, dim3((unsigned)nblk), dim3(256), 0, (hipStream_t)stream, dy, mask, x, part, nrows, H, W); break;
        default: hipLaunchKernelGGL(conv1_bwd_kernel<3>, dim3((unsigned)nblk), dim3(256), 0, (hipStream_t)stream, dy, mask, x, part, nrows, H, W); break;
    }
    HK_LAUNCH_CHECK();
    const int nel = (9 * Cin + 1) * 64;
    hipLaunchKernelGGL(partial_sum_kernel<16>, dim3((nel + 63) / 64), dim3(1024), 0, (hipStream_t)stream, (const float*)part, (int)nblk, nel,
                       9 * Cin * 64, dwt, dbias);
    HK_LAUNCH_CHECK();
    return HK_OK;
}
```

hawkeye_amd/functional.py:

```python
import contextlib
import threading

import numpy as np
import torch

from . import _lib
from ._lib import check, ptr, stream


def _f32c(t):
    if t.dtype != torch.float32:
        raise _lib.HawkeyeHipError(f'hawkeye_amd ops are fp32 (reference parity target); got {t.dtype}')
    return t.contiguous()


def _f32_shaped(t, shape, what, name):
    if tuple(t.shape) != tuple(shape):
        raise _lib.HawkeyeHipError(f'{what}: {name} must have the shape {tuple(shape)}, got {tuple(t.shape)}')
    return _f32c(t)


def _int_tensor(t, shape, dtype, device, what, name, same_device=False):
    if t.is_floating_point() or t.dtype == torch.bool:
        raise _lib.HawkeyeHipError(f'{what}: {name} must be integers; got {t.dtype}')
# ... 1678 lines not shown
        b, c, h, w = x.shape
        hw, j, k = h * w, c * c, weight.shape[0]
        if weight.shape[1] != j:
            raise _lib.HawkeyeHipError(f'bilinear_pool_linear: weight {tuple(weight.shape)} does not match {c} x {c} pooled features')
        y = torch.empty(b, j, dtype=torch.float32, device=x.device)
        inv_norm = torch.empty(b, dtype=torch.float32, device=x.device)
        colsum = torch.empty(b, hw, dtype=torch.float32, device=x.device)
        nws = lib.hk_bcnn_pool_ws_bytes(b, c, hw)
        ws = _ws(nws, x.device)
        check(lib.hk_bcnn_pool_fwd(ptr(x), ptr(y), ptr(inv_norm), ptr(colsum), b, c, hw, ptr(ws), nws, stream()),
              'hk_bcnn_pool_fwd')
        pre = torch.empty(b, k, dtype=torch.float32, device=x.device)
        nwl = lib.hk_linear_ws_bytes(b, j, k)
        wsl = _ws(nwl, x.device)
        check(lib.hk_linear_fwd(ptr(y), ptr(weight), None, ptr(pre), b, j, k, ptr(wsl), nwl, stream()), 'hk_linear_fwd')
        ctx.save_for_backward(x, y, inv_norm, colsum, weight, pre)
        ctx.has_bias = bias is not None
        return pre + _f32c(bias) if bias is not None else pre.clone()

    @staticmethod
    def backward(ctx, g):
        lib = _lib.load()
        x, y, inv_norm, colsum, weight, pre = ctx.saved_tensors
        g = _f32c(g)
        b, c, h, w = x.shape
        hw, j, k = h * w, c * c, weight.shape[0]
        need_x, need_w = ctx.needs_input_grad[0], ctx.needs_input_grad[1]
        dy = torch.empty_like(y) if need_x else None
        dw = torch.empty_like(weight) if need_w else None
        db = torch.empty(k, dtype=torch.float32, device=x.device) if (ctx.has_bias and ctx.needs_input_grad[2]) else None
        if dy is not None or dw is not None or db is not None:
            check(lib.hk_linear_bwd(ptr(y), ptr(weight), ptr(g), ptr(dy), ptr(dw), ptr(db), b, j, k, stream()), 'hk_linear_bwd')
        dx = None
        if need_x:
            dx = torch.empty_like(x)
            nws = lib.hk_bcnn_pool_ws_bytes(b, c, hw)
            ws = _ws(nws, x.device)
            check(lib.hk_bcnn_pool_bwd_tdot(ptr(x), ptr(y), ptr(dy), ptr(inv_norm), ptr(colsum), ptr(g), ptr(pre), None, k,
                                            ptr(dx), b, c, hw, ptr(ws), nws, stream()), 'hk_bcnn_pool_bwd_tdot')
        return dx, dw, db


def bilinear_pool_linear(x, weight, bias=None):
    return _BilinearPoolLinear.apply(x, weight, bias)


def ssqrt_pool_linear(x, weight, bias=None):
    return _SsqrtPoolLinear.apply(x, weight, bias)


def linear(y, weight, bias=None):
    return _Linear.apply(y, weight, bias)


def _nhwc(t, what):
    if t.dtype != torch.float32:
        raise _lib.HawkeyeHipError(f'{what}: fp32 only, got {t.dtype}')
    if t.dim() != 4 or not t.is_contiguous(memory_format=torch.channels_last):
        raise _lib.HawkeyeHipError(f'{what}: needs a channels_last [N,C,H,W] tensor, got shape {tuple(t.shape)} strides {t.stride()}')
    return t


def trunk_epilogue_ok(x, pool=False):
    if not (torch.is_tensor(x) and x.is_cuda and x.dtype == torch.float32 and x.dim() == 4):
        return False
    n, c, h, w = x.shape
    ok = n > 0 and c % 4 == 0 and c // 4 <= 256 and 256 % (c // 4) == 0 and x.is_contiguous(memory_format=torch.channels_last)
    return ok and (not pool or (h % 2 == 0 and w % 2 == 0 and h > 0 and w > 0)) and x.data_ptr() % 16 == 0


class _BiasReLU(torch.autograd.Function):

    @staticmethod
    def forward(ctx, x, bias):
        lib = _lib.load()
        _nhwc(x, 'bias_relu')
        n, c, h, w = x.shape
        b = _f32c(bias)
        mask = torch.empty(n, h, w, c // 4, dtype=torch.uint8, device=x.device) if any(ctx.needs_input_grad) else None
        check(lib.hk_bias_relu_fwd(ptr(x), ptr(b), ptr(mask), n * h * w, c, stream()), 'hk_bias_relu_fwd')
        ctx.mark_dirty(x)
        ctx.save_for_backward(mask)
        ctx.in_shape = (n, c, h, w)
        return x

    @staticmethod
    def backward(ctx, dy):
        lib = _lib.load()
        (mask,) = ctx.saved_tensors
        n, c, h, w = ctx.in_shape
        if dy.dtype != torch.float32:
            raise _lib.HawkeyeHipError(f'bias_relu backward: fp32 only, got {dy.dtype}')
        dy = dy.contiguous(memory_format=torch.channels_last)
        dx = torch.empty_like(dy, memory_format=torch.channels_last)
        db = torch.empty(c, dtype=torch.float32, device=dy.device)
        nws = lib.hk_trunk_ws_bytes(c)
        ws = _ws(nws, dy.device)
        check(lib.hk_bias_relu_bwd(ptr(dy), None, ptr(mask), ptr(dx), ptr(db), n * h * w, c, ptr(ws), nws, stream()), 'hk_bias_relu_bwd')
        return dx, db


class _BiasReLUPool(torch.autograd.Function):

    @staticmethod
    def forward(ctx, x, bias):
        lib = _lib.load()
        _nhwc(x, 'bias_relu_pool')
        n, c, h, w = x.shape
        b = _f32c(bias)
        p = torch.empty(n, c, h // 2, w // 2, dtype=torch.float32, device=x.device, memory_format=torch.channels_last)
        am = torch.empty(n, h // 2, w // 2, c // 4, dtype=torch.uint8, device=x.device)
        check(lib.hk_bias_relu_pool_fwd(ptr(x), ptr(b), ptr(p), ptr(am), n, h, w, c, stream()), 'hk_bias_relu_pool_fwd')
        ctx.save_for_backward(p, am)
        ctx.in_shape = (n, c, h, w)
        return p

    @staticmethod
    def backward(ctx, dp):
        lib = _lib.load()
        p, am = ctx.saved_tensors
        n, c, h, w = ctx.in_shape
        if dp.dtype != torch.float32:
            raise _lib.HawkeyeHipError(f'bias_relu_pool backward: fp32 only, got {dp.dtype}')
        dp = dp.contiguous(memory_format=torch.channels_last)
        dx = torch.empty(n, c, h, w, dtype=torch.float32, device=p.device, memory_format=torch.channels_last)
        db = torch.empty(c, dtype=torch.float32, device=p.device)
        nws = lib.hk_trunk_ws_bytes(c)
        ws = _ws(nws, p.device)
        check(lib.hk_bias_relu_pool_bwd(ptr(dp), ptr(p), ptr(am), ptr(dx), ptr(db), n, h, w, c, ptr(ws), nws, stream()),
              'hk_bias_relu_pool_bwd')
        return dx, db


def _same_dense_layout(a, b):
    return (a.shape == b.shape and a.stride() == b.stride() and a.dtype == b.dtype == torch.float32 and a.numel() % 4 == 0 and a.numel() > 0
            and (a.is_contiguous() or (a.dim() == 4 and a.is_contiguous(memory_format=torch.channels_last))))


def add_relu_ok(a, b):
    return torch.is_tensor(a) and torch.is_tensor(b) and a.is_cuda and b.is_cuda and _same_dense_layout(a, b) and \
        a.data_ptr() % 16 == 0 and b.data_ptr() % 16 == 0


class _AddReLU(torch.autograd.Function):

    @staticmethod
    def forward(ctx, a, b):
        lib = _lib.load()
        if not _same_dense_layout(a, b):
            raise _lib.HawkeyeHipError(f'add_relu: operands must share one dense fp32 layout, got {tuple(a.shape)} {a.stride()} / '
                                       f'{tuple(b.shape)} {b.stride()}')
        check(lib.hk_add_relu_fwd(ptr(a), ptr(b), a.numel(), stream()), 'hk_add_relu_fwd')
        ctx.mark_dirty(a)
        ctx.save_for_backward(a)
        return a

    @staticmethod
    def backward(ctx, dy):
        lib = _lib.load()
        (y,) = ctx.saved_tensors
        if dy.dtype != torch.float32:
            raise _lib.HawkeyeHipError(f'add_relu backward: fp32 only, got {dy.dtype}')
        if dy.stride() != y.stride():
            dy = dy.contiguous(memory_format=torch.channels_last) if (y.dim() == 4 and not y.is_contiguous()) else dy.contiguous()
        g = torch.empty_like(y)
        check(lib.hk_relu_mask_bwd(ptr(dy), ptr(y), ptr(g), y.numel(), stream()), 'hk_relu_mask_bwd')
        return g, g


def add_relu(a, b):
    return _AddReLU.apply(a, b)


def conv1_ok(x, conv):
    if not (torch.is_tensor(x) and x.is_cuda and x.dtype == torch.float32 and x.dim() == 4 and not x.requires_grad):
        return False
    two = lambda v: (v, v) if isinstance(v, int) else tuple(v)
    return (x.shape[1] <= 3 and conv.in_channels == x.shape[1] and conv.out_channels == 64 and conv.bias is not None
            and two(conv.kernel_size) == (3, 3) and two(conv.stride) == (1, 1) and two(conv.padding) == (1, 1)
            and two(conv.dilation) == (1, 1) and conv.groups == 1 and conv.padding_mode == 'zeros'
            and x.is_contiguous(memory_format=torch.channels_last) and x.numel() > 0)


class _Conv1BiasReLU(torch.autograd.Function):

    @staticmethod
    def forward(ctx, x, weight, bias):
        lib = _lib.load()
        _nhwc(x, 'conv1_bias_relu')
        n, cin, h, w = x.shape
        if tuple(weight.shape) != (64, cin, 3, 3):
            raise _lib.HawkeyeHipError(f'conv1_bias_relu: weight {tuple(weight.shape)} does not match [64, {cin}, 3, 3]')
        wt = weight.detach().permute(2, 3, 1, 0).reshape(9 * cin, 64).contiguous()
        b = _f32c(bias.detach())
        y = torch.empty(n, 64, h, w, dtype=torch.float32, device=x.device, memory_format=torch.channels_last)
        mask = torch.empty(n, h, w, 16, dtype=torch.uint8, device=x.device) if any(ctx.needs_input_grad[1:]) else None
        check(lib.hk_conv1_bias_relu_fwd(ptr(x), ptr(wt), ptr(b), ptr(y), ptr(mask), n, h, w, cin, 64, stream()), 'hk_conv1_bias_relu_fwd')
        ctx.save_for_backward(x, mask)
        ctx.wfmt = weight.is_contiguous(memory_format=torch.channels_last) and not weight.is_contiguous()
        return y

    @staticmethod
    def backward(ctx, dy):
        lib = _lib.load()
        x, mask = ctx.saved_tensors
        n, cin, h, w = x.shape
        if dy.dtype != torch.float32:
            raise _lib.HawkeyeHipError(f'conv1_bias_relu backward: fp32 only, got {dy.dtype}')
        dy = dy.contiguous(memory_format=torch.channels_last)
        dwt = torch.empty(9 * cin, 64, dtype=torch.float32, device=x.device)
        db = torch.empty(64, dtype=torch.float32, device=x.device)
        nws = lib.hk_conv1_ws_bytes(cin)
        ws = _ws(nws, x.device)
        check(lib.hk_conv1_bias_relu_bwd(ptr(dy), ptr(mask), ptr(x), ptr(dwt), ptr(db), n, h, w, cin, 64, ptr(ws), nws, stream()),
              'hk_conv1_bias_relu_bwd')
        dw = dwt.view(3, 3, cin, 64).permute(3, 2, 0, 1)
        dw = dw.contiguous(memory_format=torch.channels_last) if ctx.wfmt else dw.contiguous()
        return None, dw, db


def conv1_bias_relu(x, weight, bias):
    return _Conv1BiasReLU.apply(x, weight, bias)


def _two(v):
    return (v, v) if isinstance(v, int) else tuple(v)


WRW_WIDE_WINS = {
    (128, 128, 224, 224): (64, 16),
    (128, 256, 112, 112): (64, 16), (256, 256, 112, 112): (64, 16),
    (256, 512, 56, 56): (64, 16), (512, 512, 56, 56): (64, 16),
    (512, 512, 28, 28): (64, 16),
}


def _knob(name):
    import ctypes
    v = ctypes.c_int(0)
    check(_lib.load().hk_tuning_get(name, ctypes.byref(v)), f'hk_tuning_get({name.decode()})')
    return v.value


def conv3x3_wrw_route(cout, n, h, w, cin=64):
    if _knob(b'conv_wrw') == 0:
        return False
    if cin <= 64:
        return True
    split = _knob(b'wrw_split')
    if _knob(b'wrw_wide') == 0 or split == 0:
        return False
    return split > 0 or n in WRW_WIDE_WINS.get((cin, cout, h, w), ())


def _conv3x3_served(x, conv):
    if not (torch.is_tensor(x) and x.is_cuda and x.dtype == torch.float32 and x.dim() == 4 and x.numel() > 0
            and x.is_contiguous(memory_format=torch.channels_last) and x.data_ptr() % 16 == 0):
        return False
    w = conv.weight
    if not (w.dtype == torch.float32 and w.device == x.device and w.is_contiguous(memory_format=torch.channels_last)):
        return False
    return (conv.in_channels > 0 and conv.in_channels % 64 == 0 and x.shape[1] == conv.in_channels and conv.out_channels > 0
            and conv.out_channels % 64 == 0
            and _two(conv.kernel_size) == (3, 3) and _two(conv.stride) == (1, 1) and _two(conv.padding) == (1, 1)
            and _two(conv.dilation) == (1, 1) and conv.groups == 1 and conv.padding_mode == 'zeros')


def conv3x3_wrw_ok(x, conv):
    return _conv3x3_served(x, conv) and conv3x3_wrw_route(conv.out_channels, x.shape[0], x.shape[2], x.shape[3], conv.in_channels)


def conv3x3_wrw_raw(x, dy):
    lib = _lib.load()
    _nhwc(x, 'conv3x3_wrw')
    _nhwc(dy, 'conv3x3_wrw')
    n, cin, h, w = x.shape
    cout = dy.shape[1]
    if tuple(dy.shape) != (n, cout, h, w) or x.numel() == 0 or dy.numel() == 0:
        raise _lib.HawkeyeHipError(f'conv3x3_wrw: dy {tuple(dy.shape)} does not match x {tuple(x.shape)}')
    px, pdy = ptr(x), ptr(dy)
    buf = torch.empty(cout, 3, 3, cin, dtype=torch.float32, device=x.device)
    nws = lib.hk_conv3x3_wrw_ws_bytes(cin, cout)
    ws = _ws(nws, x.device)
    check(lib.hk_conv3x3_wrw(pdy, px, ptr(buf), n, h, w, cin, cout, ptr(ws), nws, stream()), 'hk_conv3x3_wrw')
    return buf.permute(0, 3, 1, 2)


def conv3x3_wrw_pooled_raw(x, dp, p, aux):
    lib = _lib.load()
    _nhwc(x, 'conv3x3_wrw_pooled')
    _nhwc(dp, 'conv3x3_wrw_pooled')
    _nhwc(p, 'conv3x3_wrw_pooled')
    n, cin, h, w = x.shape
    cout = dp.shape[1]
    if (h % 2 or w % 2 or tuple(dp.shape) != (n, cout, h // 2, w // 2) or tuple(p.shape) != tuple(dp.shape) or aux.dtype != torch.uint8
            or tuple(aux.shape) != (n, h // 2, w // 2, cout // 4) or x.numel() == 0 or dp.numel() == 0):
        raise _lib.HawkeyeHipError(f'conv3x3_wrw_pooled: dp {tuple(dp.shape)}, p {tuple(p.shape)}, codes {tuple(aux.shape)} do not match x {tuple(x.shape)}')
    px, pdp, pp, pa = ptr(x), ptr(dp), ptr(p), ptr(aux)
    buf = torch.empty(cout, 3, 3, cin, dtype=torch.float32, device=x.device)
    nws = lib.hk_conv3x3_wrw_ws_bytes(cin, cout)
    ws = _ws(nws, x.device)
    check(lib.hk_conv3x3_wrw_pooled(pdp, pp, pa, px, ptr(buf), n, h, w, cin, cout, ptr(ws), nws, stream()), 'hk_conv3x3_wrw_pooled')
    return buf.permute(0, 3, 1, 2)


CONV_FWD_WINS = {
    (64, 64, 448, 448): (64, 16), (64, 128, 224, 224): (64, 16), (128, 128, 224, 224): (64, 16),
    (128, 256, 112, 112): (64, 16), (256, 256, 112, 112): (64, 16),
    (256, 512, 56, 56): (64, 16), (512, 512, 56, 56): (64, 16),
    (512, 512, 28, 28): (64, 16),
}
CONV_BWD_DATA_WINS = {
    (64, 64, 448, 448): (64, 16), (64, 128, 224, 224): (64, 16), (128, 128, 224, 224): (64, 16),
    (128, 256, 112, 112): (64, 16), (256, 256, 112, 112): (64, 16),
    (256, 512, 56, 56): (64, 16), (512, 512, 56, 56): (64, 16),
    (512, 512, 28, 28): (64, 16),
}


def _conv3x3_route(knob, table, cin, cout, n, h, w):
    v = _knob(knob)
    if v == 0:
        return False
    return v > 0 or n in table.get((cin, cout, h, w), ())


def conv3x3_fwd_route(cin, cout, n, h, w):
    return _conv3x3_route(b'conv_fwd', CONV_FWD_WINS, cin, cout, n, h, w)


def conv3x3_bwd_data_route(cin, cout, n, h, w):
    return _conv3x3_route(b'conv_bwd_data', CONV_BWD_DATA_WINS, cin, cout, n, h, w)


def conv3x3_fwd_ok(x, conv):
    return (_conv3x3_served(x, conv) and conv.weight.data_ptr() % 16 == 0
            and conv3x3_fwd_route(conv.in_channels, conv.out_channels, x.shape[0], x.shape[2], x.shape[3]))


def conv3x3_bwd_data_ok(x, conv):
    return (_conv3x3_served(x, conv) and conv.weight.data_ptr() % 16 == 0
            and conv3x3_bwd_data_route(conv.in_channels, conv.out_channels, x.shape[0], x.shape[2], x.shape[3]))


CONV_MFMA16_FWD = {
    (256, 256, 112, 112): (64,),
    (256, 512, 56, 56): (64, 16), (512, 512, 56, 56): (64,),
    (512, 512, 28, 28): (16,),
}
CONV_MFMA16_BWD_DATA = {
    (64, 64, 448, 448): (64,),
    (128, 256, 112, 112): (64, 16), (256, 256, 112, 112): (64, 16),
    (256, 512, 56, 56): (64, 16), (512, 512, 56, 56): (64, 16),
    (512, 512, 28, 28): (16,),
}


def conv3x3_mfma_route(direction, cin, cout, n, h, w):
    v = _knob(b'conv_mfma')
    if v >= 0:
        return v == 1
    table = CONV_MFMA16_FWD if direction == 'fwd' else CONV_MFMA16_BWD_DATA
    return n in table.get((cin, cout, h, w), ())


def _conv3x3_mfma(direction, cin, cout, n, h, w):
    if _knob(b'conv_mfma') < 0 and conv3x3_mfma_route(direction, cin, cout, n, h, w):
        return _lib.tuning(conv_mfma=1)
    return contextlib.nullcontext()


def _conv3x3_call(fn, what, src, weight, cout_of_result):
    lib = _lib.load()
    _nhwc(src, what)
    if (weight.dim() != 4 or tuple(weight.shape[2:]) != (3, 3) or not weight.is_contiguous(memory_format=torch.channels_last)
            or weight.dtype != torch.float32 or weight.device != src.device):
        raise _lib.HawkeyeHipError(f'{what}: wants a channels_last fp32 [Cout, Cin, 3, 3] weight on {src.device}, got {weight.dtype} {tuple(weight.shape)}')
    n, _, h, w = src.shape
    cout, cin = weight.shape[0], weight.shape[1]
    if src.numel() == 0 or src.shape[1] != (cin if cout_of_result else cout):
        raise _lib.HawkeyeHipError(f'{what}: map {tuple(src.shape)} does not match the weight {tuple(weight.shape)}')
    psrc, pw = ptr(src), ptr(weight)
    out = torch.empty((n, cout if cout_of_result else cin, h, w), dtype=torch.float32, device=src.device, memory_format=torch.channels_last)
    nws = lib.hk_conv3x3_ws_bytes(cin, cout)
    ws = _ws(nws, src.device)
    with _conv3x3_mfma('fwd' if cout_of_result else 'bwd_data', cin, cout, n, h, w):
        check(getattr(lib, fn)(psrc, pw, ptr(out), n, h, w, cin, cout, ptr(ws), nws, stream()), fn)
    return out


def conv3x3_fwd_raw(x, weight):
    return _conv3x3_call('hk_conv3x3_fwd', 'conv3x3_fwd', x, weight, True)


def conv3x3_bwd_data_raw(dy, weight):
    return _conv3x3_call('hk_conv3x3_bwd_data', 'conv3x3_bwd_data', dy, weight, False)


class _Conv3x3(torch.autograd.Function):

    @staticmethod
    def forward(ctx, x, weight, fwd, bwd, wrw):
        ctx.save_for_backward(x, weight)
        ctx.routes = (bwd, wrw)
        if fwd:
            return conv3x3_fwd_raw(x, weight)
        return torch.nn.functional.conv2d(x, weight, None, 1, 1, 1, 1)

    @staticmethod
    def backward(ctx, dy):
        x, weight = ctx.saved_tensors
        bwd, wrw = ctx.routes
        if dy.dtype != torch.float32:
            raise _lib.HawkeyeHipError(f'conv3x3 backward: fp32 only, got {dy.dtype}')
        dy = dy.contiguous(memory_format=torch.channels_last)
        dx = dw = None
        need_dx, need_dw = ctx.needs_input_grad[0], ctx.needs_input_grad[1]
        if need_dx and bwd:
            dx = conv3x3_bwd_data_raw(dy, weight)
        if need_dw and wrw:
            dw = conv3x3_wrw_raw(x, dy)
        mask = (need_dx and not bwd, need_dw and not wrw, False)
        if mask[0] or mask[1]:
            g = torch.ops.aten.convolution_backward(dy, x, weight, None, (1, 1), (1, 1), (1, 1), False, (0, 0), 1, mask)
            dx = g[0] if mask[0] else dx
            dw = g[1] if mask[1] else dw
        return dx, dw, None, None, None


def conv3x3(x, weight, fwd=False, bwd=False, wrw=True):
    e = ConvEpilogue.take()
    if e is not None:
        if not fwd:
            raise _lib.HawkeyeHipError('conv3x3: an epilogue inside the kernel needs the forward on the kernel (fwd)')
        return _ConvUnit.apply(x, weight, e.bias, e.pool, bool(bwd), bool(wrw), e.masked, e.link_in, e.link)
    return _Conv3x3.apply(x, weight, bool(fwd), bool(bwd), bool(wrw))


def conv3x3_wrw(x, weight):
    return _Conv3x3.apply(x, weight, False, False, True)


CONV_EPI_FWD_LOSES = {}
CONV_EPI_MASKED_LOSES = {}


def conv3x3_epi_level():
    return _knob(b'conv_epi')


def conv3x3_epi_fwd_ok(x, conv, fwd):
    c = conv.out_channels
    return bool(fwd and conv3x3_epi_level() >= 1 and conv.bias is not None and conv.bias.dtype == torch.float32
                and conv.bias.data_ptr() % 16 == 0 and 256 % (c // 4) == 0
                and x.shape[0] not in CONV_EPI_FWD_LOSES.get((conv.in_channels, c, x.shape[2], x.shape[3]), ()))


def conv3x3_epi_masked_ok(x, conv, bwd):
    return bool(bwd and conv3x3_epi_level() >= 2
                and x.shape[0] not in CONV_EPI_MASKED_LOSES.get((conv.in_channels, conv.out_channels, x.shape[2], x.shape[3]), ()))


class ConvLink:
    __slots__ = ('mask', 'db')

    def __init__(self, mask=None):
        self.mask, self.db = mask, None


class _ConvUnit(torch.autograd.Function):

    @staticmethod
    def forward(ctx, x, weight, bias, pool, bwd, wrw, masked, link_in, link_out):
        lib = _lib.load()
        _nhwc(x, 'conv3x3 unit')
        n, cin, h, w = x.shape
        cout = weight.shape[0]
        if (tuple(weight.shape) != (cout, cin, 3, 3) or not weight.is_contiguous(memory_format=torch.channels_last)
                or weight.dtype != torch.float32 or weight.device != x.device):
            raise _lib.HawkeyeHipError(f'conv3x3 unit: wants a channels_last fp32 [Cout, {cin}, 3, 3] weight on {x.device}, got {weight.dtype} {tuple(weight.shape)}')
        b = _f32c(bias)
        px, pw = ptr(x), ptr(weight)
        nws = lib.hk_conv3x3_ws_bytes(cin, cout)
        ws = _ws(nws, x.device)
        grad = any(ctx.needs_input_grad[:3])
        if pool:
            y = torch.empty((n, cout, h // 2, w // 2), dtype=torch.float32, device=x.device, memory_format=torch.channels_last)
            aux = torch.empty(n, h // 2, w // 2, cout // 4, dtype=torch.uint8, device=x.device)
            with _conv3x3_mfma('fwd', cin, cout, n, h, w):
                check(lib.hk_conv3x3_bias_relu_pool_fwd(px, pw, ptr(b), ptr(y), ptr(aux), n, h, w, cin, cout, ptr(ws), nws, stream()),
                      'hk_conv3x3_bias_relu_pool_fwd')
        else:
            y = torch.empty((n, cout, h, w), dtype=torch.float32, device=x.device, memory_format=torch.channels_last)
            aux = torch.empty(n, h, w, cout // 4, dtype=torch.uint8, device=x.device) if grad else None
            with _conv3x3_mfma('fwd', cin, cout, n, h, w):
                check(lib.hk_conv3x3_bias_relu_fwd(px, pw, ptr(b), ptr(y), ptr(aux), n, h, w, cin, cout, ptr(ws), nws, stream()),
                      'hk_conv3x3_bias_relu_fwd')
            link_out.mask = aux
        min_ = link_in.mask if (masked and link_in is not None) else None
        ctx.save_for_backward(x, weight, aux, y if pool else None, min_)
        ctx.cfg = (pool, bwd, wrw, (n, cout, h, w))
        ctx.links = (link_in, link_out)
        return y

    @staticmethod
    def backward(ctx, dy):
        lib = _lib.load()
        x, weight, aux, p, min_ = ctx.saved_tensors
        pool, bwd, wrw, (n, cout, h, w) = ctx.cfg
        link_in, link_out = ctx.links
        cin = x.shape[1]
        if dy.dtype != torch.float32:
            raise _lib.HawkeyeHipError(f'conv3x3 unit backward: fp32 only, got {dy.dtype}')
        dy = dy.contiguous(memory_format=torch.channels_last)
        db, link_out.db = link_out.db, None
        if pool:
            g = torch.empty(n, cout, h, w, dtype=torch.float32, device=x.device, memory_format=torch.channels_last)
            db = torch.empty(cout, dtype=torch.float32, device=x.device)
            nws = lib.hk_trunk_ws_bytes(cout)
            ws = _ws(nws, x.device)
            check(lib.hk_bias_relu_pool_bwd(ptr(dy), ptr(p), ptr(aux), ptr(g), ptr(db), n, h, w, cout, ptr(ws), nws, stream()),
                  'hk_bias_relu_pool_bwd')
        elif db is not None:
            g = dy
        else:
            g = torch.empty_like(dy, memory_format=torch.channels_last)
            db = torch.empty(cout, dtype=torch.float32, device=x.device)
            nws = lib.hk_trunk_ws_bytes(cout)
            ws = _ws(nws, x.device)
            check(lib.hk_bias_relu_bwd(ptr(dy), None, ptr(aux), ptr(g), ptr(db), n * h * w, cout, ptr(ws), nws, stream()),
                  'hk_bias_relu_bwd')
        dx = dw = None
        need_dx, need_dw = ctx.needs_input_grad[0], ctx.needs_input_grad[1]
        if need_dx and bwd:
            if min_ is not None:
                dx = torch.empty_like(x, memory_format=torch.channels_last)
                dbp = torch.empty(cin, dtype=torch.float32, device=x.device)
                nws = lib.hk_conv3x3_masked_ws_bytes(n, h, w, cin, cout)
                ws = _ws(nws, x.device)
                with _conv3x3_mfma('bwd_data', cin, cout, n, h, w):
                    check(lib.hk_conv3x3_masked_bwd_data(ptr(g), ptr(weight), ptr(min_), ptr(dx), ptr(dbp), n, h, w, cin, cout, ptr(ws), nws,
                                                         stream()), 'hk_conv3x3_masked_bwd_data')
                link_in.db = dbp
            else:
                dx = conv3x3_bwd_data_raw(g, weight)
        if need_dw and wrw:
            if pool and lib.hk_conv3x3_wrw_pooled_served(n, h, w, cin, cout):
                dw = conv3x3_wrw_pooled_raw(x, dy, p, aux)
            else:
                dw = conv3x3_wrw_raw(x, g)
        lib_mask = (need_dx and not bwd, need_dw and not wrw, False)
        if lib_mask[0] or lib_mask[1]:
            r = torch.ops.aten.convolution_backward(g, x, weight, None, (1, 1), (1, 1), (1, 1), False, (0, 0), 1, lib_mask)
            dx = r[0] if lib_mask[0] else dx
            dw = r[1] if lib_mask[1] else dw
        return dx, dw, (db if ctx.needs_input_grad[2] else None), None, None, None, None, None, None


class ConvEpilogue:
    _pending = threading.local()

    def __init__(self, bias, pool, masked, link_in):
        self.bias, self.pool, self.masked, self.link_in, self.link = bias, bool(pool), bool(masked), link_in, ConvLink()

    def __enter__(self):
        ConvEpilogue._pending.request = self
        return self

    def __exit__(self, *exc):
        ConvEpilogue._pending.request = None
        return False

    @staticmethod
    def take():
        e = getattr(ConvEpilogue._pending, 'request', None)
        ConvEpilogue._pending.request = None
        return e


def bias_relu(x, bias):
    return _BiasReLU.apply(x, bias)


def bias_relu_pool(x, bias):
    return _BiasReLUPool.apply(x, bias)


def image_finalize(u8, erase=None, mean=(0.485, 0.456, 0.406), std=(0.229, 0.224, 0.225), channels_last=False):
    import ctypes
    lib = _lib.load()
    if u8.dtype != torch.uint8 or u8.dim() != 4 or u8.shape[3] != 3:
        raise _lib.HawkeyeHipError(f'image_finalize wants uint8 [B,H,W,3], got {u8.dtype} {tuple(u8.shape)}')
    u8 = u8.contiguous()
    b, h, w, _ = u8.shape
    fmt = torch.channels_last if channels_last else torch.contiguous_format
    out = torch.empty(b, 3, h, w, dtype=torch.float32, device=u8.device).contiguous(memory_format=fmt)
    if erase is not None:
        erase = erase.to(device=u8.device, dtype=torch.int32).contiguous()
        if erase.shape != (b, 4):
            raise _lib.HawkeyeHipError(f'image_finalize: erase boxes must be [B,4], got {tuple(erase.shape)}')
    m3, s3 = (ctypes.c_float * 3)(*mean), (ctypes.c_float * 3)(*std)
    check(lib.hk_image_finalize(ptr(u8), ctypes.cast(m3, ctypes.c_void_p), ctypes.cast(s3, ctypes.c_void_p), ptr(erase),
                                ptr(out.permute(0, 2, 3, 1) if channels_last else out), b, h, w, int(channels_last),
                                stream()), 'hk_image_finalize')
    return out


def bgemm(a, b, trans_a=False, trans_b=False, alpha=1.0, beta=0.0, diag=0.0, out=None):
    lib = _lib.load()
    a, b = _f32c(a), _f32c(b)
    nb = a.shape[0]
    m, k = (a.shape[2], a.shape[1]) if trans_a else (a.shape[1], a.shape[2])
    n = b.shape[1] if trans_b else b.shape[2]
    if out is None:
        out = torch.zeros(nb, m, n, dtype=torch.float32, device=a.device)
    check(lib.hk_bgemm_f32(ptr(a), a.shape[2], a.shape[1] * a.shape[2], int(trans_a),
                           ptr(b), b.shape[2], b.shape[1] * b.shape[2], int(trans_b),
                           ptr(out), n, m * n, m, n, k, nb, float(alpha), float(beta), float(diag), stream()),
          'hk_bgemm_f32')
    return out
```

include/hawkeye_conv_pool.h:

```cpp
#ifndef HAWKEYE_CONV_POOL_H
#define HAWKEYE_CONV_POOL_H

#include <stddef.h>
#include <stdint.h>

#include "hawkeye_hip.h"

#ifdef __cplusplus
extern "C" {
#endif

int hk_conv3x3_wrw_pooled(const float* dp, const float* p, const uint8_t* argmax, const float* x, float* dw, int N, int H, int W, int Cin,
                          int Cout, void* ws, size_t ws_bytes, hk_stream_t stream);

int hk_conv3x3_wrw_pooled_served(int N, int H, int W, int Cin, int Cout);

int hk_conv3x3_wrw_pooled_plan(int N, int H, int W, int Cin, int Cout, int* out);

#ifdef __cplusplus
}
#endif

#endif
```

Baseline: 660.7 images/sec.

## Fuse maxpool and ReLU backward into conv3x3 bwd-data input staging

```diff
diff --git a/hawkeye_amd/_lib.py b/hawkeye_amd/_lib.py
--- a/hawkeye_amd/_lib.py
+++ b/hawkeye_amd/_lib.py
@@ -141,6 +141,10 @@
     'hk_conv3x3_wrw_pooled': (c_i, [c_f, c_f, c_f, c_f, c_f, c_i, c_i, c_i, c_i, c_i, c_f, c_sz, c_f]),
     'hk_conv3x3_wrw_pooled_served': (c_i, [c_i] * 5),
     'hk_conv3x3_wrw_pooled_plan': (c_i, [c_i] * 5 + [c_f]),
+    'hk_conv3x3_bwd_pooled_ws_bytes': (c_sz, [c_i] * 5),
+    'hk_conv3x3_bwd_data_pooled': (c_i, [c_f] * 6 + [c_i] * 5 + [c_f, c_sz, c_f]),
+    'hk_conv3x3_masked_bwd_data_pooled': (c_i, [c_f] * 8 + [c_i] * 5 + [c_f, c_sz, c_f]),
+    'hk_conv3x3_bwd_pooled_served': (c_i, [c_i] * 5),
 }
 
 INTERP_SIGNATURES = {
diff --git a/hawkeye_amd/csrc/api.hip b/hawkeye_amd/csrc/api.hip
--- a/hawkeye_amd/csrc/api.hip
+++ b/hawkeye_amd/csrc/api.hip
@@ -25,7 +25,7 @@
     {"conv_fwd", "HK_CONV_FWD", &Tuning::conv_fwd},             {"conv_bwd_data", "HK_CONV_BWD_DATA", &Tuning::conv_bwd_data},
     {"conv_epi", "HK_CONV_EPI", &Tuning::conv_epi},             {"conv_mfma", "HK_CONV_MFMA", &Tuning::conv_mfma},
     {"wrw_mfma", "HK_WRW_MFMA", &Tuning::wrw_mfma},             {"conv_tile", "HK_CONV_TILE", &Tuning::conv_tile},
-    {"wrw_pool", "HK_WRW_POOL", &Tuning::wrw_pool},
+    {"wrw_pool", "HK_WRW_POOL", &Tuning::wrw_pool},             {"bwd_pool", "HK_BWD_POOL", &Tuning::bwd_pool},
 };
 Tuning from_env() {
     Tuning t;
diff --git a/hawkeye_amd/csrc/conv_fwd.hip b/hawkeye_amd/csrc/conv_fwd.hip
--- a/hawkeye_amd/csrc/conv_fwd.hip
+++ b/hawkeye_amd/csrc/conv_fwd.hip
@@ -155,6 +155,12 @@
 }
 
 constexpr int CF_EPI_NONE = 0, CF_EPI_RELU = 1, CF_EPI_POOL = 2, CF_EPI_MASK = 3;
+constexpr int CF_SRC_MAP = 0, CF_SRC_POOLED = 1;
+#if defined(__HIP_DEVICE_COMPILE__)
+#define CF_LOAD1_ASYNC(dst, ptr) asm volatile("global_load_ubyte %0, %1, off" : "=v"(dst) : "v"(ptr) : "memory")
+#else
+#define CF_LOAD1_ASYNC(dst, ptr) ((dst) = *(ptr))
+#endif
 constexpr int CF_PARK = CF_CO + 4;
 constexpr int CF_DB_RPG = 128;
 static_assert(CF_R * CF_SW * CF_PARK * 4 <= CF_LDS, "the parked tile fits the LDS of the main loop");
@@ -265,13 +271,15 @@
     }
 }
 
-template <int EPI, int MF, int G>
+template <int EPI, int MF, int G, int SRC = CF_SRC_MAP>
 __device__ __forceinline__ void conv3x3_split_tile(float* ldsf, const float* __restrict__ x, const char* __restrict__ ws, float* __restrict__ y,
                                                    int H, int W, int Cin, int Cout, long long n, int r0, int c0, int tile, int cot,
-                                                   const float* __restrict__ bias, uint8_t* __restrict__ mk, double* __restrict__ part) {
+                                                   const float* __restrict__ bias, uint8_t* __restrict__ mk, double* __restrict__ part,
+                                                   const float* __restrict__ pool_p = nullptr, const uint8_t* __restrict__ pool_am = nullptr) {
     typedef CfGeo<G> GE;
     constexpr bool M32 = MF == CF_MF_32;
     static_assert(!(M32 && G == CF_G_16x8), "16 x 8 is a geometry of CF_MF_16 only");
+    static_assert(SRC == CF_SRC_MAP || (!M32 && (EPI == CF_EPI_NONE || EPI == CF_EPI_MASK)), "the pooled source: CF_MF_16, the two input gradients");
     constexpr int XPLANE = cf_xplane<MF, G>(), WTAP = M32 ? CF_WTAP : CF16_WTAP;
     constexpr int XU = GE::XU, XF4 = GE::XF4, HC = GE::HC, HP = GE::HP;
     char* xs = reinterpret_cast<char*>(ldsf);
@@ -280,11 +288,27 @@
     const int l15 = lane & 15, kg = lane >> 4;
     const int wave = __builtin_amdgcn_readfirstlane(tid >> 6);
     const int nchunk = Cin / CF_CK, total = nchunk * 9;
-    const float* xi = x + n * H * W * Cin;
+    const float* xi = x + (SRC == CF_SRC_MAP ? n * H * W * Cin : n * (H / 2) * (W / 2) * Cin);
     const char* wt = ws + (size_t)cot * total * WTAP + tid * 16;
 
-    long long xoff[XU];
+    constexpr int WR = GE::TH / 2 + 2, WC = GE::TW / 2 + 2, WF4 = WR * WC * (CF_CK / 4), WU = (WF4 + 255) / 256;
+    constexpr int NX = SRC == CF_SRC_MAP ? XU : WU;
+    constexpr int XREQ = SRC == CF_SRC_MAP ? XU : 3 * WU;
+    long long xoff[NX];
     unsigned xok = 0;
+    if constexpr (SRC == CF_SRC_POOLED) {
+        const int Ho = H / 2, Wo = W / 2;
+#pragma unroll
+        for (int u = 0; u < WU; ++u) {
+            const int idx = tid + 256 * u;
+            const bool in = idx < WF4;
+            const int wd = in ? idx >> 3 : 0, wr = wd / WC, wc = wd - wr * WC;
+            const int row = r0 / 2 - 1 + wr, col = c0 / 2 - 1 + wc;
+            if (in && row >= 0 && row < Ho && col >= 0 && col < Wo) xok |= 1u << u;
+            const int rc = row < 0 ? 0 : (row < Ho ? row : Ho - 1), cc = col < 0 ? 0 : (col < Wo ? col : Wo - 1);
+            xoff[u] = ((long long)rc * Wo + cc) * Cin + 4 * (idx & 7);
+        }
+    } else {
 #pragma unroll
     for (int u = 0; u < XU; ++u) {
         const int idx = tid + 256 * u;
@@ -295,6 +319,7 @@
         const int rc = row < 0 ? 0 : (row < H ? row : H - 1), cc = col < 0 ? 0 : (col < W ? col : W - 1);
         xoff[u] = ((long long)rc * W + cc) * Cin + 4 * (idx & 7);
     }
+    }
     const int xdst = M32 ? (tid >> 3) * CF_PIX + (tid & 7) * 8 : cf16_off(tid >> 3, (tid & 7) >> 1) + (tid & 1) * 8;
     auto xdst_of = [&](int u) {
         if constexpr (HP == HC) {
@@ -305,11 +330,31 @@
         }
     };
 
-    f32x4 vx[XU];
+    f32x4 vx[NX], vp[SRC == CF_SRC_MAP ? 1 : WU];
+    unsigned vc[SRC == CF_SRC_MAP ? 1 : WU];
     auto load_x = [&](int chunk) {
         const float* b = xi + chunk * CF_CK;
-#pragma unroll
-        for (int u = 0; u < XU; ++u) HK_LOAD16_ASYNC(vx[u], b + xoff[u]);
+        if constexpr (SRC == CF_SRC_MAP) {
+#pragma unroll
+            for (int u = 0; u < XU; ++u) HK_LOAD16_ASYNC(vx[u], b + xoff[u]);
+        } else {
+            const float* bp = pool_p + n * (H / 2) * (W / 2) * Cin + chunk * CF_CK;
+            const uint8_t* bc = pool_am + n * (H / 2) * (W / 2) * (Cin / 4) + chunk * (CF_CK / 4);
+#pragma unroll
+            for (int u = 0; u < WU; ++u) {
+                HK_LOAD16_ASYNC(vx[u], b + xoff[u]);
+                HK_LOAD16_ASYNC(vp[u], bp + xoff[u]);
+                CF_LOAD1_ASYNC(vc[u], bc + (xoff[u] >> 2));
+            }
+        }
+    };
+    auto pin_x = [&]() {
+#pragma unroll
+        for (int u = 0; u < NX; ++u) {
+            HK_PIN_LOADED(vx[u]);
+            HK_PIN_LOADED(vp[u]);
+            HK_PIN_LOADED(vc[u]);
+        }
     };
     auto load_w = [&](int it, int buf) {
         const char* b = wt + (size_t)it * WTAP;
@@ -320,7 +365,47 @@
             if (wave < 3) glds16(reinterpret_cast<const float*>(b + 3 * 4096), reinterpret_cast<float*>(d + 3 * 4096));
         }
     };
+    unsigned pd[SRC == CF_SRC_MAP ? 1 : WU][2];
+    if constexpr (SRC == CF_SRC_POOLED) {
+#pragma unroll
+        for (int u = 0; u < WU; ++u) {
+            const int wd = (tid >> 3) + 32 * u, wr = wd / WC, wc = wd - wr * WC;
+#pragma unroll
+            for (int dh = 0; dh < 2; ++dh) {
+                pd[u][dh] = 0;
+#pragma unroll
+                for (int j = 0; j < 2; ++j) {
+                    const int hr = 2 * wr + dh - 1, hc = 2 * wc + (j ^ ((tid >> 4) & 1)) - 1;
+                    const bool ok = tid + 256 * u < WF4 && hr >= 0 && hr < GE::HR && hc >= 0 && hc < HC;
+                    pd[u][dh] |= (ok ? (unsigned)(cf16_off(hr * HP + hc, (tid & 7) >> 1) + (tid & 1) * 8) : 0xffffu) << (16 * j);
+                }
+            }
+        }
+    }
     auto store_x = [&]() {
+        if constexpr (SRC == CF_SRC_POOLED) {
+            typedef unsigned u32x2 __attribute__((ext_vector_type(2)));
+            const unsigned swap = (tid >> 4) & 1;
+#pragma unroll
+            for (int u = 0; u < WU; ++u) {
+                f32x4 d;
+#pragma unroll
+                for (int t = 0; t < 4; ++t) d[t] = (((xok >> u) & 1) && !(vp[u][t] <= 0.f)) ? vx[u][t] : 0.f;
+                bf16x4 p[3];
+                wrs_split(d, p);
+#pragma unroll
+                for (int k = 0; k < 4; ++k) {
+                    const unsigned off = (pd[u][k >> 1] >> (16 * (k & 1))) & 0xffffu;
+                    if (off != 0xffffu) {
+                        const unsigned e = vc[u] ^ (((unsigned)(k >> 1) * 0xaau) | (((unsigned)(k & 1) ^ swap) * 0x55u)), z = ~(e | (e >> 1));
+                        auto all = [&](int bit) { return (unsigned)-(int)((z >> bit) & 1u); };
+                        const u32x2 m = {(all(0) & 0xffffu) | (all(2) << 16), (all(4) & 0xffffu) | (all(6) << 16)};
+#pragma unroll
+                        for (int sp = 0; sp < 3; ++sp) *reinterpret_cast<u32x2*>(xs + sp * XPLANE + off) = __builtin_bit_cast(u32x2, p[sp]) & m;
+                    }
+                }
+            }
+        } else {
         const f32x4 zero = {0.f, 0.f, 0.f, 0.f};
 #pragma unroll
         for (int u = 0; u < XU; ++u) {
@@ -332,6 +417,7 @@
                 for (int s = 0; s < 3; ++s) *reinterpret_cast<bf16x4*>(xs + s * XPLANE + d) = p[s];
             }
         }
+        }
     };
 
     f32x16 acc[2], sum[2];
@@ -353,8 +439,12 @@
     load_w(0, 0);
     load_x(0);
     __builtin_amdgcn_s_waitcnt(HK_VMCNT_IMM(0));
+    if constexpr (SRC == CF_SRC_MAP) {
 #pragma unroll
     for (int u = 0; u < XU; ++u) HK_PIN_LOADED(vx[u]);
+    } else {
+        pin_x();
+    }
     store_x();
     HK_LDS_BARRIER();
 
@@ -416,11 +506,15 @@
 #pragma unroll
                         for (int pb = 0; pb < 2; ++pb) acc4[cb][pb] = mfma_f32_16x16x32_bf16(a[cb][PA[pr]], b[pb][PB[pr]], acc4[cb][pb]);
             }
-            if (tap == 5) CF_TAP_BARRIER(XU);
+            if (tap == 5) CF_TAP_BARRIER(XREQ);
             else CF_TAP_BARRIER(0);
             if (tap == 6) {
+                if constexpr (SRC == CF_SRC_MAP) {
 #pragma unroll
                 for (int u = 0; u < XU; ++u) HK_PIN_LOADED(vx[u]);
+                } else {
+                    pin_x();
+                }
             }
             if (tap == 8 && more) {
                 store_x();
@@ -596,6 +690,34 @@
     }
 }
 
+template <int EPI, int MF, int PLAN, int SRC>
+__device__ __forceinline__ void conv3x3_split_block(const float* __restrict__ x, const char* __restrict__ ws, float* __restrict__ y, int H, int W,
+                                                    int Cin, int Cout, int nstrips, int nrb, int ntiles, const float* __restrict__ bias,
+                                                    uint8_t* __restrict__ mk, double* __restrict__ part, int nstripsB, int tpi,
+                                                    const float* __restrict__ pool_p, const uint8_t* __restrict__ pool_am) {
+    HK_DYN_LDS16(ldsf);
+    int tile, cot;
+    if (!xcd_map(blockIdx.x, ntiles, Cout / CF_CO, tile, cot)) return;
+    if constexpr (PLAN != CF_PLAN_MIXED) {
+        typedef CfGeo<PLAN> GE;
+        const int strip = tile % nstrips, tr = tile / nstrips;
+        const int rb = tr % nrb;
+        const long long n = tr / nrb;
+        conv3x3_split_tile<EPI, MF, PLAN, SRC>(ldsf, x, ws, y, H, W, Cin, Cout, n, rb * GE::TH, strip * GE::TW, tile, cot, bias, mk, part, pool_p,
+                                               pool_am);
+    } else {
+        const long long n = tile / tpi;
+        const int t = tile % tpi, nA = nrb * nstrips;
+        if (t < nA) {
+            conv3x3_split_tile<EPI, MF, CF_G_8x16, SRC>(ldsf, x, ws, y, H, W, Cin, Cout, n, (t / nstrips) * 8, (t % nstrips) * 16, tile, cot, bias, mk,
+                                                        part, pool_p, pool_am);
+        } else {
+            const int tb = t - nA;
+            conv3x3_split_tile<EPI, MF, CF_G_16x8, SRC>(ldsf, x, ws, y, H, W, Cin, Cout, n, (tb / nstripsB) * 16, nstrips * 16 + (tb % nstripsB) * 8,
+                                                        tile, cot, bias, mk, part, pool_p, pool_am);
+        }
+    }
+}
 template <int EPI, int MF, int PLAN>
 __global__ __launch_bounds__(256, 2) void conv3x3_split_kernel(const float* __restrict__ x, const char* __restrict__ ws,
                                                                float* __restrict__ y, int H, int W, int Cin, int Cout, int nstrips,
@@ -623,6 +745,14 @@
         }
     }
 }
+template <int EPI, int PLAN>
+__global__ __launch_bounds__(256, 2) void conv3x3_split_pooled_kernel(const float* __restrict__ dp, const float* __restrict__ p,
+                                                                      const uint8_t* __restrict__ am, const char* __restrict__ ws,
+                                                                      float* __restrict__ y, int H, int W, int Cin, int Cout, int nstrips,
+                                                                      int nrb, int ntiles, uint8_t* __restrict__ mk, double* __restrict__ part,
+                                                                      int nstripsB, int tpi) {
+    conv3x3_split_block<EPI, CF_MF_16, PLAN, CF_SRC_POOLED>(dp, ws, y, H, W, Cin, Cout, nstrips, nrb, ntiles, nullptr, mk, part, nstripsB, tpi, p, am);
+}
 
 template <int Q, typename OUT>
 __global__ __launch_bounds__(64 * Q) void conv3x3_colsum_kernel(const double* __restrict__ part, int nrows, int nel, int rpg,
@@ -713,6 +843,32 @@
     return conv3x3_run_on<EPI, CF_MF_32, CF_PLAN_4x32>(x, w, y, N, H, W, K, M, transposed, ws, stream, bias, mk, part, pl);
 }
 
+template <int EPI, int PLAN>
+static int conv3x3_run_pooled_on(const float* dp, const float* p, const uint8_t* am, const float* w, float* y, int N, int H, int W, int K, int M,
+                                 void* ws, hipStream_t stream, uint8_t* mk, double* part, const CfPlan& pl) {
+    constexpr int LDS = cf_lds<CF_MF_16, PLAN>();
+    const long long ntiles = N * pl.tpi;
+    const int ncot = M / CF_CO;
+    if ((ntiles + NXCD) * ncot > 0x7fffffffll) return HK_ERR_UNSUPPORTED;
+    const long long total = (long long)ncot * (K / CF_CK) * 9 * CF_CO * 8;
+    hipLaunchKernelGGL(conv3x3_wsplit_kernel<CF_MF_16>, dim3((unsigned)((total + 255) / 256)), dim3(256), 0, stream, w, (char*)ws, M, K, 1, total);
+    HK_LAUNCH_CHECK();
+    HK_ALLOW_BIG_LDS((conv3x3_split_pooled_kernel<EPI, PLAN>), LDS);
+    hipLaunchKernelGGL((conv3x3_split_pooled_kernel<EPI, PLAN>), dim3((unsigned)xcd_grid((int)ntiles, ncot)), dim3(256), LDS, stream, dp, p, am,
+                       (const char*)ws, y, H, W, K, M, pl.nstrips, pl.nrb, (int)ntiles, mk, part, pl.nstripsB, (int)pl.tpi);
+    HK_LAUNCH_CHECK();
+    return HK_OK;
+}
+template <int EPI>
+static int conv3x3_run_pooled(const float* dp, const float* p, const uint8_t* am, const float* w, float* y, int N, int H, int W, int K, int M,
+                              void* ws, hipStream_t stream, uint8_t* mk = nullptr, double* part = nullptr) {
+    const CfPlan pl = conv3x3_plan(H, W, CF_MF_16, tuning().conv_tile);
+    if (pl.tpi > 0x7fffffffll) return HK_ERR_UNSUPPORTED;
+    if (pl.plan == CF_PLAN_MIXED) return conv3x3_run_pooled_on<EPI, CF_PLAN_MIXED>(dp, p, am, w, y, N, H, W, K, M, ws, stream, mk, part, pl);
+    if (pl.plan == CF_PLAN_8x16) return conv3x3_run_pooled_on<EPI, CF_PLAN_8x16>(dp, p, am, w, y, N, H, W, K, M, ws, stream, mk, part, pl);
+    return conv3x3_run_pooled_on<EPI, CF_PLAN_4x32>(dp, p, am, w, y, N, H, W, K, M, ws, stream, mk, part, pl);
+}
+
 static int conv3x3_check(const float* x, const float* w, float* y, int N, int H, int W, int Cin, int Cout, void* ws, size_t ws_bytes,
                          int knob) {
     if (!x || !w || !y || N <= 0 || H <= 0 || W <= 0 || Cin <= 0 || Cout <= 0) return HK_ERR_BAD_ARG;
@@ -727,6 +883,43 @@
     return (long long)N * (((long long)H + CF_R - 1) / CF_R) * (((long long)W + CF_SW - 1) / CF_SW);
 }
 static long long conv3x3_groups(long long ntiles) { return ntiles > CF_DB_RPG ? (ntiles + CF_DB_RPG - 1) / CF_DB_RPG : 0; }
+
+static int conv3x3_colsum(double* part, long long ntiles, long long ngroups, int C, float* dbias, hipStream_t stream) {
+    double* grp = part + ntiles * C;
+    const dim3 cols((unsigned)(C / 64));
+    if (ngroups > 0) {
+        hipLaunchKernelGGL((conv3x3_colsum_kernel<16, double>), dim3(cols.x, (unsigned)ngroups), dim3(1024), 0, stream, (const double*)part,
+                           (int)ntiles, C, CF_DB_RPG, grp);
+        HK_LAUNCH_CHECK();
+        hipLaunchKernelGGL((conv3x3_colsum_kernel<16, float>), cols, dim3(1024), 0, stream, (const double*)grp, (int)ngroups, C, (int)ngroups, dbias);
+    } else {
+        hipLaunchKernelGGL((conv3x3_colsum_kernel<16, float>), cols, dim3(1024), 0, stream, (const double*)part, (int)ntiles, C, (int)ntiles, dbias);
+    }
+    HK_LAUNCH_CHECK();
+    return HK_OK;
+}
+
+static bool bwd_pool_wins(int N, int H, int W, int Cin, int Cout) {
+    (void)Cin; (void)Cout;
+    return (long long)H * W >= 224ll * 224 && (long long)N * H * W >= 16ll * 224 * 224;
+}
+static bool bwd_pooled_shape_ok(int N, int H, int W, int Cin, int Cout) {
+    if (N <= 0 || H <= 0 || W <= 0 || Cin <= 0 || Cout <= 0) return false;
+    if (Cin % 64 != 0 || Cout % 64 != 0 || Cout > 1024 || (long long)Cout * 9 * Cin > 0x7fffffffll || H % 2 != 0 || W % 2 != 0) return false;
+    return tuning().conv_bwd_data != 0 && conv3x3_mf(N, H, W, Cout, Cin) == CF_MF_16;
+}
+static int bwd_pooled_check(const float* dp, const float* p, const uint8_t* am, const float* w, float* dx, float* dbias, int N, int H, int W, int Cin,
+                            int Cout, void* ws, size_t ws_bytes) {
+    if (!dp || !p || !am || !w || !dx || !dbias || N <= 0 || H <= 0 || W <= 0 || Cin <= 0 || Cout <= 0) return HK_ERR_BAD_ARG;
+    if (!ws || ws_bytes < hk_conv3x3_bwd_pooled_ws_bytes(N, H, W, Cin, Cout)) return HK_ERR_WORKSPACE;
+    if (!bwd_pooled_shape_ok(N, H, W, Cin, Cout) || tuning().bwd_pool == 0 || !aligned16(dp) || !aligned16(p) || !aligned16(am) || !aligned16(w) ||
+        !aligned16(dx) || !aligned16(ws))
+        return HK_ERR_UNSUPPORTED;
+    return HK_OK;
+}
+static int bwd_pooled_db(const float* dp, const float* p, float* dbias, int N, int H, int W, int Cin, int Cout, void* ws, hipStream_t stream) {
+    return trunk_pool_db(dp, p, dbias, (long long)N * (H / 2) * (W / 2), Cout, (char*)ws + hk_conv3x3_masked_ws_bytes(N, H, W, Cin, Cout), stream);
+}
 
 }
 
@@ -800,20 +993,41 @@
     const long long ntiles = N * conv3x3_plan(H, W, conv3x3_mf(N, H, W, Cout, Cin), tuning().conv_tile).tpi, ngroups = conv3x3_groups(ntiles);
     if (ntiles > conv3x3_tiles(N, H, W) || ntiles > 0x7fffffffll || ngroups > 65535) return HK_ERR_UNSUPPORTED;
     double* part = reinterpret_cast<double*>((char*)ws + hk_conv3x3_ws_bytes(Cin, Cout));
-    double* grp = part + ntiles * Cin;
     const int rc2 = conv3x3_run<CF_EPI_MASK>(dy, w, dx, N, H, W, Cout, Cin, true, ws, (hipStream_t)stream, nullptr, const_cast<uint8_t*>(mask), part);
     if (rc2 != HK_OK) return rc2;
-    const dim3 cols((unsigned)(Cin / 64));
-    if (ngroups > 0) {
-        hipLaunchKernelGGL((conv3x3_colsum_kernel<16, double>), dim3(cols.x, (unsigned)ngroups), dim3(1024), 0, (hipStream_t)stream,
-                           (const double*)part, (int)ntiles, Cin, CF_DB_RPG, grp);
-        HK_LAUNCH_CHECK();
-        hipLaunchKernelGGL((conv3x3_colsum_kernel<16, float>), cols, dim3(1024), 0, (hipStream_t)stream, (const double*)grp, (int)ngroups, Cin,
-                           (int)ngroups, dbias);
-    } else {
-        hipLaunchKernelGGL((conv3x3_colsum_kernel<16, float>), cols, dim3(1024), 0, (hipStream_t)stream, (const double*)part, (int)ntiles, Cin,
-                           (int)ntiles, dbias);
-    }
-    HK_LAUNCH_CHECK();
-    return HK_OK;
-}
+    return conv3x3_colsum(part, ntiles, ngroups, Cin, dbias, (hipStream_t)stream);
+}
+
+extern "C" size_t hk_conv3x3_bwd_pooled_ws_bytes(int N, int H, int W, int Cin, int Cout) {
+    if (N <= 0 || H <= 0 || W <= 0 || Cin <= 0 || Cout <= 0) return 0;
+    return hk_conv3x3_masked_ws_bytes(N, H, W, Cin, Cout) + hk_trunk_ws_bytes(Cout);
+}
+
+extern "C" int hk_conv3x3_bwd_pooled_served(int N, int H, int W, int Cin, int Cout) {
+    const int pool = tuning().bwd_pool;
+    if (pool == 0 || !bwd_pooled_shape_ok(N, H, W, Cin, Cout)) return 0;
+    return pool > 0 || bwd_pool_wins(N, H, W, Cin, Cout) ? 1 : 0;
+}
+
+extern "C" int hk_conv3x3_bwd_data_pooled(const float* dp, const float* p, const uint8_t* argmax, const float* w, float* dx, float* dbias, int N,
+                                          int H, int W, int Cin, int Cout, void* ws, size_t ws_bytes, hk_stream_t stream) {
+    const int rc = bwd_pooled_check(dp, p, argmax, w, dx, dbias, N, H, W, Cin, Cout, ws, ws_bytes);
+    if (rc != HK_OK) return rc;
+    const int rc2 = conv3x3_run_pooled<CF_EPI_NONE>(dp, p, argmax, w, dx, N, H, W, Cout, Cin, ws, (hipStream_t)stream);
+    return rc2 != HK_OK ? rc2 : bwd_pooled_db(dp, p, dbias, N, H, W, Cin, Cout, ws, (hipStream_t)stream);
+}
+
+extern "C" int hk_conv3x3_masked_bwd_data_pooled(const float* dp, const float* p, const uint8_t* argmax, const float* w, const uint8_t* mask,
+                                                 float* dx, float* dbias_producer, float* dbias, int N, int H, int W, int Cin, int Cout, void* ws,
+                                                 size_t ws_bytes, hk_stream_t stream) {
+    if (!mask || !dbias_producer) return HK_ERR_BAD_ARG;
+    const int rc = bwd_pooled_check(dp, p, argmax, w, dx, dbias, N, H, W, Cin, Cout, ws, ws_bytes);
+    if (rc != HK_OK) return rc;
+    if (!aligned16(mask) || tuning().conv_epi < 2) return HK_ERR_UNSUPPORTED;
+    const long long ntiles = N * conv3x3_plan(H, W, CF_MF_16, tuning().conv_tile).tpi, ngroups = conv3x3_groups(ntiles);
+    if (ntiles > conv3x3_tiles(N, H, W) || ntiles > 0x7fffffffll || ngroups > 65535) return HK_ERR_UNSUPPORTED;
+    double* part = reinterpret_cast<double*>((char*)ws + hk_conv3x3_ws_bytes(Cin, Cout));
+    int rc2 = conv3x3_run_pooled<CF_EPI_MASK>(dp, p, argmax, w, dx, N, H, W, Cout, Cin, ws, (hipStream_t)stream, const_cast<uint8_t*>(mask), part);
+    if (rc2 == HK_OK) rc2 = conv3x3_colsum(part, ntiles, ngroups, Cin, dbias_producer, (hipStream_t)stream);
+    return rc2 != HK_OK ? rc2 : bwd_pooled_db(dp, p, dbias, N, H, W, Cin, Cout, ws, (hipStream_t)stream);
+}
diff --git a/hawkeye_amd/csrc/hk_common.h b/hawkeye_amd/csrc/hk_common.h
--- a/hawkeye_amd/csrc/hk_common.h
+++ b/hawkeye_amd/csrc/hk_common.h
@@ -51,6 +51,7 @@
     int wrw_wide = 1;
     int wrw_mfma = -1;
     int wrw_pool = -1;
+    int bwd_pool = -1;
     int conv_fwd = -1;
     int conv_bwd_data = -1;
     int conv_epi = 2;
@@ -59,6 +60,7 @@
     int peer_form = 0;
 };
 Tuning& tuning();
+int trunk_pool_db(const float* dp, const float* p, float* dbias, long long npix, int C, void* ws, hipStream_t stream);
 
 constexpr int HK_MAX_AUX = 3;
 struct AuxQueue {
diff --git a/hawkeye_amd/csrc/trunk.hip b/hawkeye_amd/csrc/trunk.hip
--- a/hawkeye_amd/csrc/trunk.hip
+++ b/hawkeye_amd/csrc/trunk.hip
@@ -193,6 +193,34 @@
     trunk_db_partial(acc, part, c4);
 }
 
+__global__ __launch_bounds__(256) void pool_db_kernel(const float* __restrict__ dp, const float* __restrict__ p, float* __restrict__ part,
+                                                      long long npix, long long ppb, int c4) {
+    const int tid = threadIdx.x, q = tid % c4, r0 = tid / c4, rstep = 256 / c4;
+    const long long pbeg = (long long)blockIdx.x * ppb, pend = pbeg + ppb < npix ? pbeg + ppb : npix;
+    const f32x4* dp4 = reinterpret_cast<const f32x4*>(dp);
+    const f32x4* p4 = reinterpret_cast<const f32x4*>(p);
+    f32x4 acc = (f32x4){0.f, 0.f, 0.f, 0.f};
+    if (r0 < rstep) {
+        for (long long pix = pbeg + r0; pix < pend; pix += 4 * rstep) {
+            f32x4 g[4], v[4];
+#pragma unroll
+            for (int u = 0; u < 4; ++u) {
+                const long long pp = pix + u * rstep;
+                if (pp < pend) { g[u] = dp4[pp * c4 + q]; v[u] = p4[pp * c4 + q]; }
+            }
+#pragma unroll
+            for (int u = 0; u < 4; ++u) {
+                if (pix + u * rstep >= pend) continue;
+                f32x4 d;
+#pragma unroll
+                for (int t = 0; t < 4; ++t) d[t] = !(v[u][t] <= 0.f) ? g[u][t] : 0.f;
+                acc += d;
+            }
+        }
+    }
+    trunk_db_partial(acc, part, c4);
+}
+
 __global__ __launch_bounds__(256) void add_relu_fwd_kernel(float* __restrict__ a, const float* __restrict__ b, long long n4) {
     f32x4* a4 = reinterpret_cast<f32x4*>(a);
     const f32x4* b4 = reinterpret_cast<const f32x4*>(b);
@@ -236,6 +264,17 @@
 static inline int trunk_blocks(long long rows) {
     long long b = (rows + 63) / 64;
     return (int)(b < 1 ? 1 : (b > TRUNK_PART_BLOCKS ? TRUNK_PART_BLOCKS : b));
+}
+
+int trunk_pool_db(const float* dp, const float* p, float* dbias, long long npix, int C, void* ws, hipStream_t stream) {
+    if (C < 4 || C % 4 != 0 || C / 4 > 256 || !aligned16(ws)) return HK_ERR_UNSUPPORTED;
+    const int nblk = trunk_blocks(npix);
+    const long long ppb = (npix + nblk - 1) / nblk;
+    hipLaunchKernelGGL(pool_db_kernel, dim3(nblk), dim3(256), 0, stream, dp, p, (float*)ws, npix, ppb, C / 4);
+    HK_LAUNCH_CHECK();
+    hipLaunchKernelGGL(trunk_db_final_kernel, dim3((C + 15) / 16), dim3(256), 0, stream, (const float*)ws, nblk, C, dbias);
+    HK_LAUNCH_CHECK();
+    return HK_OK;
 }
 
 }
diff --git a/hawkeye_amd/functional.py b/hawkeye_amd/functional.py
--- a/hawkeye_amd/functional.py
+++ b/hawkeye_amd/functional.py
@@ -2004,6 +2004,35 @@
     ws = _ws(nws, x.device)
     check(lib.hk_conv3x3_wrw_pooled(pdp, pp, pa, px, ptr(buf), n, h, w, cin, cout, ptr(ws), nws, stream()), 'hk_conv3x3_wrw_pooled')
     return buf.permute(0, 3, 1, 2)
+
+
+def conv3x3_bwd_data_pooled_raw(dp, p, aux, weight, mask=None):
+    lib = _lib.load()
+    _nhwc(dp, 'conv3x3_bwd_data_pooled')
+    _nhwc(p, 'conv3x3_bwd_data_pooled')
+    n, cout, ho, wo = dp.shape
+    cin = weight.shape[1]
+    h, w = 2 * ho, 2 * wo
+    if (tuple(weight.shape) != (cout, cin, 3, 3) or not weight.is_contiguous(memory_format=torch.channels_last) or weight.dtype != torch.float32
+            or tuple(p.shape) != tuple(dp.shape) or aux.dtype != torch.uint8 or tuple(aux.shape) != (n, ho, wo, cout // 4) or dp.numel() == 0
+            or (mask is not None and (mask.dtype != torch.uint8 or tuple(mask.shape) != (n, h, w, cin // 4)))):
+        raise _lib.HawkeyeHipError(f'conv3x3_bwd_data_pooled: dp {tuple(dp.shape)}, p {tuple(p.shape)}, codes {tuple(aux.shape)} and the weight '
+                                   f'{tuple(weight.shape)} do not match')
+    pdp, pp, pa, pw, pm = ptr(dp), ptr(p), ptr(aux), ptr(weight), ptr(mask)
+    dx = torch.empty((n, cin, h, w), dtype=torch.float32, device=dp.device, memory_format=torch.channels_last)
+    db = torch.empty(cout, dtype=torch.float32, device=dp.device)
+    nws = lib.hk_conv3x3_bwd_pooled_ws_bytes(n, h, w, cin, cout)
+    ws = _ws(nws, dp.device)
+    dbp = None
+    with _conv3x3_mfma('bwd_data', cin, cout, n, h, w):
+        if mask is None:
+            check(lib.hk_conv3x3_bwd_data_pooled(pdp, pp, pa, pw, ptr(dx), ptr(db), n, h, w, cin, cout, ptr(ws), nws, stream()),
+                  'hk_conv3x3_bwd_data_pooled')
+        else:
+            dbp = torch.empty(cin, dtype=torch.float32, device=dp.device)
+            check(lib.hk_conv3x3_masked_bwd_data_pooled(pdp, pp, pa, pw, pm, ptr(dx), ptr(dbp), ptr(db), n, h, w, cin, cout, ptr(ws), nws,
+                                                        stream()), 'hk_conv3x3_masked_bwd_data_pooled')
+    return dx, (dbp, db)
 
 
 CONV_FWD_WINS = {
@@ -2216,6 +2245,14 @@
             raise _lib.HawkeyeHipError(f'conv3x3 unit backward: fp32 only, got {dy.dtype}')
         dy = dy.contiguous(memory_format=torch.channels_last)
         db, link_out.db = link_out.db, None
+        need_dx, need_dw = ctx.needs_input_grad[0], ctx.needs_input_grad[1]
+        if (pool and need_dx and bwd and lib.hk_conv3x3_bwd_pooled_served(n, h, w, cin, cout)
+                and (not need_dw or (wrw and lib.hk_conv3x3_wrw_pooled_served(n, h, w, cin, cout)))):
+            dx, dbp = conv3x3_bwd_data_pooled_raw(dy, p, aux, weight, min_)
+            if min_ is not None:
+                link_in.db = dbp[0]
+            dw = conv3x3_wrw_pooled_raw(x, dy, p, aux) if need_dw else None
+            return dx, dw, (dbp[1] if ctx.needs_input_grad[2] else None), None, None, None, None, None, None
         if pool:
             g = torch.empty(n, cout, h, w, dtype=torch.float32, device=x.device, memory_format=torch.channels_last)
             db = torch.empty(cout, dtype=torch.float32, device=x.device)
@@ -2233,7 +2270,6 @@
             check(lib.hk_bias_relu_bwd(ptr(dy), None, ptr(aux), ptr(g), ptr(db), n * h * w, cout, ptr(ws), nws, stream()),
                   'hk_bias_relu_bwd')
         dx = dw = None
-        need_dx, need_dw = ctx.needs_input_grad[0], ctx.needs_input_grad[1]
         if need_dx and bwd:
             if min_ is not None:
                 dx = torch.empty_like(x, memory_format=torch.channels_last)
diff --git a/include/hawkeye_conv_pool.h b/include/hawkeye_conv_pool.h
--- a/include/hawkeye_conv_pool.h
+++ b/include/hawkeye_conv_pool.h
@@ -17,6 +17,15 @@
 
 int hk_conv3x3_wrw_pooled_plan(int N, int H, int W, int Cin, int Cout, int* out);
 
+size_t hk_conv3x3_bwd_pooled_ws_bytes(int N, int H, int W, int Cin, int Cout);
+int hk_conv3x3_bwd_data_pooled(const float* dp, const float* p, const uint8_t* argmax, const float* w, float* dx, float* dbias, int N, int H,
+                               int W, int Cin, int Cout, void* ws, size_t ws_bytes, hk_stream_t stream);
+int hk_conv3x3_masked_bwd_data_pooled(const float* dp, const float* p, const uint8_t* argmax, const float* w, const uint8_t* mask, float* dx,
+                                      float* dbias_producer, float* dbias, int N, int H, int W, int Cin, int Cout, void* ws, size_t ws_bytes,
+                                      hk_stream_t stream);
+
+int hk_conv3x3_bwd_pooled_served(int N, int H, int W, int Cin, int Cout);
+
 #ifdef __cplusplus
 }
 #endif
```

Result: no change. 664.6 images/sec, median of 6 (+0.6%).
